# phazei/ComfyUI-HunyuanVideo-Foley

Hardware: AMD Instinct MI355X
Metric: audio-sec/sec (5s clip, 50-step Euler, CFG 4.5) (higher is better)
Workload: dtype bf16; 1 GPU; c2: T2A 5 s, 50 Euler steps, CFG 4.5, hunyuanvideo-foley-xxl, bs=1/GPU, bf16 GEMM operands / fp32 accumulate, weight storage none, DAC-VAE fp32 decode to 48 kHz, host-to-host (H2D noise + D2H waveform timed); clips_per_gpu=1, parallelism=dp1, hip_graph=True, progress_callback=False, collectives=0, bundle_bytes=10565004032, rccl_nranks=1

## Files before the change

### comfyui-hunyuanvideo-foley_amd/csrc/attention.hip

```cpp
#include <type_traits>

#include "kernels.h"

namespace {


template <int HD> __device__ constexpr float attn_scale() {
  return HD == 128 ? 0.08838834764831845f : HD == 64 ? 0.125f : 0.10206207261596575f;
}

__device__ __forceinline__ void attn_block_coords(const AttnArgs& a, int qtile, int& qt, int& h, int& b) {
  const int nq = (a.Sq + qtile - 1) / qtile;
  const int nwg = nq * a.H * a.Bq;
  int bid = (int)blockIdx.x;
  const int xcd = bid & 7, slot = bid >> 3;
  const int q = nwg >> 3, r = nwg & 7;
  bid = ((xcd < r) ? xcd * (q + 1) : r * (q + 1) + (xcd - r) * q) + slot;
  qt = bid % nq;
  const int bh = bid / nq;
  h = bh % a.H;
  b = bh / a.H;
}

template <typename OutT> struct Pack4Out;
template <> struct Pack4Out<float> {
  static __device__ __forceinline__ void store(float* p, const f32x4 v) { *(f32x4*)p = v; }
};
template <> struct Pack4Out<bf16_t> {
  static __device__ __forceinline__ void store(bf16_t* p, const f32x4 v) {
    uint2 w;
    w.x = pack_bf16x2(v[0], v[1]);
    w.y = pack_bf16x2(v[2], v[3]);
    *(uint2*)p = w;
  }
};

template <> struct Pack4Out<f16_t> {
  static __device__ __forceinline__ void store(f16_t* p, const f32x4 v) {
    uint2 w;
    w.x = pack_f16x2(v[0], v[1]);
    w.y = pack_f16x2(v[2], v[3]);
    *(uint2*)p = w;
  }
};

template <typename OutT, int HD>
__global__ __launch_bounds__(64) void attn_kernel(const AttnArgs a) {
  const int lane = threadIdx.x;
  const int j = lane & 31, kh = lane >> 5;
  const int q0 = blockIdx.x * 32;
  const int h = blockIdx.y, b = blockIdx.z;
  const int bk = b / a.kv_bdiv;
  const float* __restrict__ Q = (const float*)a.q + ((long)(b * a.H + h) * a.Sq) * HD;
  const float* __restrict__ K = (const float*)a.k + ((long)(bk * a.H + h) * a.Skv) * HD;
  const float* __restrict__ V = (const float*)a.v + ((long)(bk * a.H + h) * a.Skv) * HD;
  const float scale = attn_scale<HD>();

  constexpr int HH = HD / 2, NC = HD / 8;
  float qr[HH];
  {
    const int qrow = min(q0 + j, a.Sq - 1);
    const f32x4* p = (const f32x4*)(Q + (long)qrow * HD + kh * HH);
#pragma unroll
    for (int c = 0; c < NC; ++c) {
      const f32x4 v = p[c];
      qr[c * 4 + 0] = v[0]; qr[c * 4 + 1] = v[1]; qr[c * 4 + 2] = v[2]; qr[c * 4 + 3] = v[3];
    }
  }

  constexpr int ND = HD / 32;
  f32x16 o[ND];
#pragma unroll
  for (int d = 0; d < ND; ++d)
#pragma unroll
    for (int e = 0; e < 16; ++e) o[d][e] = 0.f;
  float m_run = -INFINITY, l_run = 0.f;

  for (int kt = 0; kt < a.Skv; kt += 32) {
    f32x16 s;
#pragma unroll
    for (int e = 0; e < 16; ++e) s[e] = 0.f;
    {
      const int krow = min(kt + j, a.Skv - 1);
      const f32x4* p = (const f32x4*)(K + (long)krow * HD + kh * HH);
#pragma unroll
      for (int c = 0; c < NC; ++c) {
        const f32x4 v = p[c];
        s = __builtin_amdgcn_mfma_f32_32x32x2f32(v[0], qr[c * 4 + 0], s, 0, 0, 0);
        s = __builtin_amdgcn_mfma_f32_32x32x2f32(v[1], qr[c * 4 + 1], s, 0, 0, 0);
        s = __builtin_amdgcn_mfma_f32_32x32x2f32(v[2], qr[c * 4 + 2], s, 0, 0, 0);
        s = __builtin_amdgcn_mfma_f32_32x32x2f32(v[3], qr[c * 4 + 3], s, 0, 0, 0);
      }
    }
    float mx = -INFINITY;
#pragma unroll
    for (int e = 0; e < 16; ++e) {
      const int key = kt + (e & 3) + 8 * (e >> 2) + 4 * kh;
      s[e] = (key < a.Skv) ? s[e] * scale : -INFINITY;
      mx = fmaxf(mx, s[e]);
    }
    mx = xhalf_max(mx);
    const float m_new = fmaxf(m_run, mx);
    const float alpha = expf(m_run - m_new);
    float ps = 0.f;
#pragma unroll
    for (int e = 0; e < 16; ++e) {
      s[e] = expf(s[e] - m_new);
      ps += s[e];
    }
    ps = xhalf_sum(ps);
    l_run = l_run * alpha + ps;
    m_run = m_new;
#pragma unroll
    for (int d = 0; d < ND; ++d)
#pragma unroll
      for (int e = 0; e < 16; ++e) o[d][e] *= alpha;
#pragma unroll
    for (int t = 0; t < 16; ++t) {
      const int vrow = min(kt + (t & 3) + 8 * (t >> 2) + 4 * kh, a.Skv - 1);
      const float* vp = V + (long)vrow * HD + j;
#pragma unroll
      for (int d = 0; d < ND; ++d)
        o[d] = __builtin_amdgcn_mfma_f32_32x32x2f32(vp[d * 32], s[t], o[d], 0, 0, 0);
    }
  }

  const int tok = q0 + j;
  if (tok >= a.Sq) return;
  const float inv = 1.0f / l_run;
  OutT* dst;
  if (HD == 64 && a.out_rows) {
    const int orow = a.out_rows[(long)b * a.Sq + tok];
    if ((unsigned)orow >= (unsigned)a.out_nrows) return;
    dst = (OutT*)a.outA + (long)orow * (a.H * HD);
  }
  else if (tok < a.split) dst = (OutT*)a.outA + ((long)b * a.split + tok) * (a.H * HD);
  else dst = (OutT*)a.outB + ((long)b * (a.Sq - a.split) + (tok - a.split)) * (a.H * HD);
  dst += h * HD;
#pragma unroll
  for (int d = 0; d < ND; ++d)
#pragma unroll
    for (int g4 = 0; g4 < 4; ++g4) {
      const int c = d * 32 + 8 * g4 + 4 * kh;
#pragma unroll
      for (int u = 0; u < 4; ++u) dst[c + u] = Cvt<OutT>::to(o[d][g4 * 4 + u] * inv);
    }
}

template <typename T, typename OutT>
__global__ __launch_bounds__(256) void attn_bf16_kernel(const AttnArgs a) {
  constexpr int HD = 128;
  __shared__ float sO[4][3][16][64];
  __shared__ float sM[4][32], sL[4][32];
  const int lane = threadIdx.x & 63, w = threadIdx.x >> 6;
  const int j = lane & 31, kh = lane >> 5;
  int qt, h, b;
  attn_block_coords(a, 32, qt, h, b);
  const int q0 = qt * 32;
  const int bk = b / a.kv_bdiv;
  const T* __restrict__ Q = (const T*)a.q + ((long)(b * a.H + h) * a.Sq) * HD;
  const T* __restrict__ K = (const T*)a.k + ((long)(bk * a.H + h) * a.Skv) * HD;
  const T* __restrict__ VT = (const T*)a.v + ((long)(bk * a.H + h) * HD) * a.vt_pitch;
  const float scale2 = 0.08838834764831845f * 1.4426950408889634f;

  const bool stamp = a.dbg && threadIdx.x == 0;
  if (stamp) a.dbg[(long)blockIdx.x * 8 + 0] = wall_clock64();
  bf16x8 qf[8];
  {
    const T* p = Q + (long)min(q0 + j, a.Sq - 1) * HD + 8 * kh;
#pragma unroll
    for (int s = 0; s < 8; ++s) qf[s] = *(const bf16x8*)(p + 16 * s);
  }
  f32x16 o[4];
#pragma unroll
  for (int d = 0; d < 4; ++d)
#pragma unroll
    for (int e = 0; e < 16; ++e) o[d][e] = 0.f;
  float m_run = -INFINITY, l_run = 0.f;

  const int nt = (a.Skv + 31) >> 5;
  const int t0 = (nt * w) >> 2, t1 = (nt * (w + 1)) >> 2;
  const int pi = 16 * ((j >> 2) & 1) + (j & 3) + 4 * (j >> 3);
  auto tile = [&](int kt, const bf16x8 (&kf)[8], const bf16x8 (&vf)[2][4]) {
    f32x16 s;
#pragma unroll
    for (int e = 0; e < 16; ++e) s[e] = 0.f;
#pragma unroll
    for (int st = 0; st < 8; ++st) s = mfma16<T>(kf[st], qf[st], s);
    float mx = -INFINITY;
#pragma unroll
    for (int e = 0; e < 16; ++e) {
      s[e] = (kt + 16 * kh + e < a.Skv) ? s[e] * scale2 : -INFINITY;
      mx = fmaxf(mx, s[e]);
    }
    mx = xhalf_max(mx);
    const float m_new = fmaxf(m_run, mx);
    float ps = 0.f;
    bf16x8 pb[2];
#pragma unroll
    for (int e = 0; e < 16; ++e) {
      const float pv = __builtin_amdgcn_exp2f(s[e] - m_new);
      ps += pv;
      pb[e >> 3][e & 7] = to_carrier<T>(pv);
    }
    ps = xhalf_sum(ps);
    if (__builtin_amdgcn_ballot_w64(m_new > m_run) != 0) {
      const float alpha = __builtin_amdgcn_exp2f(m_run - m_new);
      l_run *= alpha;
#pragma unroll
      for (int d = 0; d < 4; ++d)
#pragma unroll
        for (int e = 0; e < 16; ++e) o[d][e] *= alpha;
    }
    l_run += ps;
    m_run = m_new;
#pragma unroll
    for (int u = 0; u < 2; ++u)
#pragma unroll
      for (int d = 0; d < 4; ++d) o[d] = mfma16<T>(vf[u][d], pb[u], o[d]);
  };
  auto load_k = [&](int kt, bf16x8 (&kf)[8]) {
    const T* p = K + (long)min(kt + pi, a.Skv - 1) * HD + 8 * kh;
#pragma unroll
    for (int st = 0; st < 8; ++st) kf[st] = *(const bf16x8*)(p + 16 * st);
  };
  auto load_v = [&](int kt, bf16x8 (&vf)[2][4]) {
#pragma unroll
    for (int u = 0; u < 2; ++u)
#pragma unroll
      for (int d = 0; d < 4; ++d) vf[u][d] = *(const bf16x8*)(VT + (long)(d * 32 + j) * a.vt_pitch + kt + 16 * kh + 8 * u);
  };
  if (t1 - t0 <= 2) {
    bf16x8 k0[8], k1[8], v0[2][4], v1[2][4];
// ... 13 lines not shown
  } else {
    for (int t = t0; t < t1; ++t) {
      bf16x8 kf[8], vf[2][4];
      load_k(t * 32, kf);
      load_v(t * 32, vf);
      tile(t * 32, kf, vf);
    }
  }

  if (stamp) a.dbg[(long)blockIdx.x * 8 + 2] = wall_clock64();
  if (kh == 0) {
    sM[w][j] = m_run;
    sL[w][j] = l_run;
  }
#pragma unroll
  for (int d = 0; d < 4; ++d) {
    if (d == w) continue;
    const int slot = d < w ? d : d - 1;
#pragma unroll
    for (int e = 0; e < 16; ++e) sO[w][slot][e][lane] = o[d][e];
  }
  __syncthreads();
  if (stamp) a.dbg[(long)blockIdx.x * 8 + 3] = wall_clock64();
  float mstar = -INFINITY;
#pragma unroll
  for (int x = 0; x < 4; ++x) mstar = fmaxf(mstar, sM[x][j]);
  float wt[4], L = 0.f;
#pragma unroll
  for (int x = 0; x < 4; ++x) {
    wt[x] = __builtin_amdgcn_exp2f(sM[x][j] - mstar);
    L += wt[x] * sL[x][j];
  }
  const int tok = q0 + j;
  if (tok >= a.Sq) return;
  const float inv = 1.0f / L;
  OutT* dst;
  if (tok < a.split) dst = (OutT*)a.outA + ((long)b * a.split + tok) * (a.H * HD);
  else dst = (OutT*)a.outB + ((long)b * (a.Sq - a.split) + (tok - a.split)) * (a.H * HD);
  dst += h * HD + w * 32;
  const int slot_mine = 0;
  (void)slot_mine;
  auto finish = [&](auto wc) {
    constexpr int W = decltype(wc)::value;
    float part[3][16];
#pragma unroll
    for (int x = 0, n = 0; x < 4; ++x) {
      if (x == W) continue;
      const int slot = W < x ? W : W - 1;
#pragma unroll
      for (int e = 0; e < 16; ++e) part[n][e] = sO[x][slot][e][lane];
      ++n;
    }
#pragma unroll
    for (int g4 = 0; g4 < 4; ++g4) {
      f32x4 r;
#pragma unroll
      for (int u = 0; u < 4; ++u) {
        const int e = g4 * 4 + u;
        float acc = 0.f;
#pragma unroll
        for (int x = 0, n = 0; x < 4; ++x) {
          if (x == W) acc += wt[x] * o[W][e];
          else acc += wt[x] * part[n++][e];
        }
        r[u] = acc * inv;
      }
      Pack4Out<OutT>::store(dst + 8 * g4 + 4 * kh, r);
    }
  };
  switch (__builtin_amdgcn_readfirstlane(w)) {
    case 0: finish(std::integral_constant<int, 0>{}); break;
    case 1: finish(std::integral_constant<int, 1>{}); break;
    case 2: finish(std::integral_constant<int, 2>{}); break;
    default: finish(std::integral_constant<int, 3>{}); break;
  }
  if (stamp) a.dbg[(long)blockIdx.x * 8 + 4] = wall_clock64();
}

__device__ __forceinline__ void attn_buf_lds16(const void* base, unsigned bytes, unsigned char* lds_wave_base, int voff) {
  const __amdgpu_buffer_rsrc_t r = __builtin_amdgcn_make_buffer_rsrc((void*)base, 0, (int)bytes, 0x00020000);
  __builtin_amdgcn_raw_ptr_buffer_load_lds(r, (__attribute__((address_space(3))) void*)lds_wave_base, 16, voff, 0, 0, 0);
}

template <typename T, typename OutT>
__global__ __launch_bounds__(256) void attn_lds_kernel(const AttnArgs a, const int merge_off) {
  constexpr int HD = 128;
  extern __shared__ __attribute__((aligned(16))) unsigned char dsm[];
  float (*sO)[3][16][64] = (float (*)[3][16][64])(dsm + merge_off);
  float (*sM)[32] = (float (*)[32])(dsm + merge_off + 4 * 3 * 16 * 64 * 4);
  float (*sL)[32] = (float (*)[32])(dsm + merge_off + 4 * 3 * 16 * 64 * 4 + 4 * 32 * 4);
  const int lane = threadIdx.x & 63, w = threadIdx.x >> 6;
  const int j = lane & 31, kh = lane >> 5;
  int qt, h, b;
  attn_block_coords(a, 32, qt, h, b);
  const int q0 = qt * 32;
  const int bk = b / a.kv_bdiv;
  const T* __restrict__ Q = (const T*)a.q + ((long)(b * a.H + h) * a.Sq) * HD;
  const T* __restrict__ K = (const T*)a.k + ((long)(bk * a.H + h) * a.Skv) * HD;
  const T* __restrict__ VT = (const T*)a.v + ((long)(bk * a.H + h) * HD) * a.vt_pitch;
  const float scale2 = 0.08838834764831845f * 1.4426950408889634f;

  const bool stamp = a.dbg && threadIdx.x == 0;
  if (stamp) a.dbg[(long)blockIdx.x * 8 + 0] = wall_clock64();
  const int nt = (a.Skv + 31) >> 5;
  const int lgCV = a.vt_pitch > 128 ? 5 : 4;
  unsigned char* const Ks = dsm;
  unsigned char* const Vs = Ks + nt * 32 * 256;
  unsigned char* const Qs = Vs + (128 << (lgCV + 4));
  const int wv = __builtin_amdgcn_readfirstlane(w);
  {
    const int r4 = lane >> 4, c16 = lane & 15;
    for (int p = wv; p < nt * 8; p += 4) {
      const int row = 4 * p + r4;
      const int g = c16 ^ ((row & 7) | ((row >> 1) & 8));
      attn_buf_lds16(K, (unsigned)a.Skv * 256u, Ks + p * 1024, row * 256 + g * 16);
    }
    const int vchunks = a.vt_pitch >> 3;
    for (int p = wv; p < (128 << lgCV) >> 6; p += 4) {
      const int pos = p * 64 + lane;
      const int row = pos >> lgCV, g = (pos & ((1 << lgCV) - 1)) ^ (row & 15);
      attn_buf_lds16(VT, (unsigned)(HD * a.vt_pitch * 2), Vs + p * 1024, g < vchunks ? (row * a.vt_pitch + g * 8) * 2 : 0x7ffffff0);
    }
    for (int p = wv; p < 8; p += 4) {
      const int row = 4 * p + r4;
      attn_buf_lds16(Q + (long)q0 * HD, (unsigned)(a.Sq - q0) * 256u, Qs + p * 1024, row * 256 + ((c16 ^ (row & 15)) << 4));
    }
  }
  asm volatile("s_waitcnt vmcnt(0)" ::: "memory");
  __syncthreads();
  if (stamp) a.dbg[(long)blockIdx.x * 8 + 1] = wall_clock64();
  bf16x8 qf[8];
#pragma unroll
  for (int s = 0; s < 8; ++s) qf[s] = *(const bf16x8*)(Qs + j * 256 + (((2 * s + kh) ^ (j & 15)) << 4));
  f32x16 o[4];
#pragma unroll
  for (int d = 0; d < 4; ++d)
#pragma unroll
    for (int e = 0; e < 16; ++e) o[d][e] = 0.f;
  float m_run = -INFINITY, l_run = 0.f;

  const int t0 = (nt * w) >> 2, t1 = (nt * (w + 1)) >> 2;
  const int pi = 16 * ((j >> 2) & 1) + (j & 3) + 4 * (j >> 3);
  auto tile = [&](int kt, const bf16x8 (&kf)[8], const bf16x8 (&vf)[2][4]) {
    f32x16 s;
#pragma unroll
    for (int e = 0; e < 16; ++e) s[e] = 0.f;
#pragma unroll
    for (int st = 0; st < 8; ++st) s = mfma16<T>(kf[st], qf[st], s);
    float mx = -INFINITY;
#pragma unroll
    for (int e = 0; e < 16; ++e) {
      s[e] = (kt + 16 * kh + e < a.Skv) ? s[e] * scale2 : -INFINITY;
      mx = fmaxf(mx, s[e]);
    }
    mx = xhalf_max(mx);
    const float m_new = fmaxf(m_run, mx);
    float ps = 0.f;
    bf16x8 pb[2];
#pragma unroll
    for (int e = 0; e < 16; ++e) {
      const float pv = __builtin_amdgcn_exp2f(s[e] - m_new);
      ps += pv;
      pb[e >> 3][e & 7] = to_carrier<T>(pv);
    }
    ps = xhalf_sum(ps);
    if (__builtin_amdgcn_ballot_w64(m_new > m_run) != 0) {
      const float alpha = __builtin_amdgcn_exp2f(m_run - m_new);
      l_run *= alpha;
// ... 523 lines not shown
      pb[e >> 3][e & 7] = to_carrier<T>(pv);
    }
    ps = xhalf_sum(ps);
    if (__builtin_amdgcn_ballot_w64(m_new > m_run) != 0) {
      const float alpha = __builtin_amdgcn_exp2f(m_run - m_new);
      l_run *= alpha;
#pragma unroll
      for (int d = 0; d < ND; ++d)
#pragma unroll
        for (int e = 0; e < 16; ++e) o[d][e] *= alpha;
    }
    l_run += ps;
    m_run = m_new;
#pragma unroll
    for (int u = 0; u < 2; ++u)
#pragma unroll
      for (int d = 0; d < ND; ++d)
        o[d] = mfma16<T>(*(const bf16x8*)(Vs + (d * 32 + j) * VP + (16 * kh + 8 * u) * 2), pb[u], o[d]);
  };
  gload(0);
  lstore(0);
  __syncthreads();
  for (int t = 0; t < nt; ++t) {
    if (t + 1 < nt) gload(t + 1);
    if (t * KT + 32 * kh2 < a.Skv) {
      qk(t & 1);
      softmax_pv(t, t & 1);
    }
    if (t + 1 < nt) {
      lstore((t + 1) & 1);
      __syncthreads();
    }
  }
  __syncthreads();
  float* xm = (float*)lds + qb * (66 * 64);
  if (kh2 == 1) {
    xm[lane] = m_run;
    xm[64 + lane] = l_run;
#pragma unroll
    for (int d = 0; d < ND; ++d)
#pragma unroll
      for (int v = 0; v < 4; ++v) {
        const f32x4 t4 = {o[d][4 * v], o[d][4 * v + 1], o[d][4 * v + 2], o[d][4 * v + 3]};
        *(f32x4*)(xm + 128 + ((d * 4 + v) * 64 + lane) * 4) = t4;
      }
  }
  __syncthreads();
  if (kh2 == 1) return;
  {
    const float m_b = xm[lane], l_b = xm[64 + lane];
    const float m = fmaxf(m_run, m_b);
    const float fa = __builtin_amdgcn_exp2f(m_run - m), fb = __builtin_amdgcn_exp2f(m_b - m);
    l_run = l_run * fa + l_b * fb;
#pragma unroll
    for (int d = 0; d < ND; ++d)
#pragma unroll
      for (int v = 0; v < 4; ++v) {
        const f32x4 t4 = *(const f32x4*)(xm + 128 + ((d * 4 + v) * 64 + lane) * 4);
#pragma unroll
        for (int e = 0; e < 4; ++e) o[d][4 * v + e] = o[d][4 * v + e] * fa + t4[e] * fb;
      }
  }
  const int tok = q0 + j;
  if (tok >= a.Sq) return;
  const float inv = 1.0f / l_run;
  OutT* dst;
  if (tok < a.split) dst = (OutT*)a.outA + ((long)b * a.split + tok) * (a.H * HD);
  else dst = (OutT*)a.outB + ((long)b * (a.Sq - a.split) + (tok - a.split)) * (a.H * HD);
  dst += h * HD;
#pragma unroll
  for (int d = 0; d < ND; ++d)
#pragma unroll
    for (int g4 = 0; g4 < 4; ++g4) {
      const f32x4 v = {o[d][g4 * 4 + 0] * inv, o[d][g4 * 4 + 1] * inv, o[d][g4 * 4 + 2] * inv, o[d][g4 * 4 + 3] * inv};
      Pack4Out<OutT>::store(dst + d * 32 + 8 * g4 + 4 * kh, v);
    }
}

}

static long long* g_attn_dbg = nullptr;
extern "C" void foley_debug_attn_timeline(void* p) { g_attn_dbg = (long long*)p; }

int launch_attention(const AttnArgs& a_in, int out_dtype, hipStream_t st) {
  AttnArgs a = a_in;
  a.dbg = g_attn_dbg;
  if (a.Sq <= 0 || a.Skv <= 0) return foley_set_err("attention: empty sequence", __FILE__, __LINE__);
  const int hd = a.head_dim > 0 ? a.head_dim : 128;
  if (hd != 128 && hd != 64 && hd != 96) return foley_set_err("attention: head_dim must be 128, 96 or 64", __FILE__, __LINE__);
  if (a.grp_q > 0 || a.grp_kv > 0) {
    if (hd != 64 || !foley_is_half(a.in_dtype) || a.grp_q < 1 || a.grp_kv < 1 || a.kv_bdiv != 1 ||
        (long)((a.Sq + a.grp_q - 1) / a.grp_q) * a.grp_kv > a.Skv)
      return foley_set_err("attention: grouped (block-diagonal) form: head_dim 64, 16-bit operands, every query group's keys inside Skv", __FILE__, __LINE__);
  }
  if (a.out_rows && hd != 64) return foley_set_err("attention: the output row table serves head_dim 64 (the conditioning encoders' kernels)", __FILE__, __LINE__);
  dim3 grid((a.Sq + 31) / 32, a.H, a.Bq), block(64);
  const dim3 grid1(grid.x * grid.y * grid.z);
  if (foley_is_half(a.in_dtype)) {
    if (a.vt_pitch < ((a.Skv + 31) & ~31) || (a.vt_pitch & 7))
      return foley_set_err("attention: V^T pitch must cover Skv rounded up to 32 (multiple of 8)", __FILE__, __LINE__);
    if (out_dtype != a.in_dtype && out_dtype != FOLEY_F32)
      return foley_set_err("attention: 16-bit operands produce the same type or fp32", __FILE__, __LINE__);
    const dim3 gw(((a.Sq + 127) / 128) * a.H * a.Bq);
    const bool wide = (long)gw.x >= 256 || hd != 128, h16 = a.in_dtype == FOLEY_F16, o32 = out_dtype == FOLEY_F32;
    const bool longk = wide && hd == 128 && a.Skv >= 512 && (long)gw.x * 4 <= 2048;
    int pair_nq = 0;
    if (longk) {
      long best = 0;
      for (int nq = 6; nq >= 4; --nq) {
        const long wgs = (long)((a.Sq + 32 * nq - 1) / (32 * nq)) * a.H * a.Bq;
        if (wgs <= 256 && wgs > best) { best = wgs; pair_nq = nq; }
      }
      if (best < 160) pair_nq = 0;
    }
    const int nt = (a.Skv + 31) >> 5;
    const long img = (long)nt * 32 * 256 + (128L << ((a.vt_pitch > 128 ? 5 : 4) + 4)) + 32 * 256, mrg = 4 * 3 * 16 * 64 * 4 + 2 * 4 * 32 * 4;
    const bool staged = !wide && hd == 128 && nt >= 4 && a.vt_pitch <= 256 && img <= 160 * 1024;
    const int merge_off = staged && img + mrg <= 160 * 1024 ? (int)img : 0;
    const size_t lds16 = staged ? (size_t)(merge_off ? img + mrg : (img > mrg ? img : mrg)) : 0;
#define FOLEY_ATTN16(T, O)                                                                         \
    do {                                                                                             \
      if (staged) {                                                                                  \
        static std::atomic<unsigned long long> raised{0};                                            \
        hipError_t e_ = foley_raise_lds((const void*)attn_lds_kernel<T, O>, 160 * 1024, raised);     \
        if (e_ != hipSuccess) return foley_set_err(hipGetErrorString(e_), __FILE__, __LINE__);       \
        FOLEY_LAUNCH((attn_lds_kernel<T, O>), grid1, dim3(256), lds16, st, a, merge_off);            \
      } else                                                                                         \
      if (pair_nq) {                                                                                 \
        static std::atomic<unsigned long long> r4{0}, r5{0}, r6{0};                                  \
        const dim3 gp(((a.Sq + 32 * pair_nq - 1) / (32 * pair_nq)) * a.H * a.Bq);                    \
        hipError_t e_ = hipSuccess;                                                                  \
        if (pair_nq == 6) { e_ = foley_raise_lds((const void*)attn_bf16_pair_kernel<T, O, 6>, 6 * 16896, r6); if (e_ == hipSuccess) FOLEY_LAUNCH((attn_bf16_pair_kernel<T, O, 6>), gp, dim3(768), 6 * 16896, st, a); } \
        else if (pair_nq == 5) { e_ = foley_raise_lds((const void*)attn_bf16_pair_kernel<T, O, 5>, 5 * 16896, r5); if (e_ == hipSuccess) FOLEY_LAUNCH((attn_bf16_pair_kernel<T, O, 5>), gp, dim3(640), 5 * 16896, st, a); } \
        else { e_ = foley_raise_lds((const void*)attn_bf16_pair_kernel<T, O, 4>, 2 * 35840, r4); if (e_ == hipSuccess) FOLEY_LAUNCH((attn_bf16_pair_kernel<T, O, 4>), gp, dim3(512), 2 * 35840, st, a); } \
        if (e_ != hipSuccess) return foley_set_err(hipGetErrorString(e_), __FILE__, __LINE__);       \
      } else                                                                                         \
      if (longk) {                                                                                   \
        static std::atomic<unsigned long long> raised{0};                                            \
        hipError_t e_ = foley_raise_lds((const void*)attn_bf16_long_kernel<T, O>, 2 * 35840, raised); \
        if (e_ != hipSuccess) return foley_set_err(hipGetErrorString(e_), __FILE__, __LINE__);       \
        FOLEY_LAUNCH((attn_bf16_long_kernel<T, O>), gw, dim3(256), 2 * 35840, st, a);                \
      } else                                                                                         \
      if (wide && hd == 64 && a.grp_q > 0) FOLEY_LAUNCH((attn_bf16_wide_kernel<T, O, 64, true>), gw, dim3(256), 0, st, a);  \
      else if (wide && hd == 64) FOLEY_LAUNCH((attn_bf16_wide_kernel<T, O, 64>), gw, dim3(256), 0, st, a);  \
      else if (wide && hd == 96) FOLEY_LAUNCH((attn_bf16_wide_kernel<T, O, 96>), gw, dim3(256), 0, st, a);  \
      else if (wide) FOLEY_LAUNCH((attn_bf16_wide_kernel<T, O, 128>), gw, dim3(256), 0, st, a);        \
      else FOLEY_LAUNCH((attn_bf16_kernel<T, O>), grid1, dim3(256), 0, st, a);                         \
    } while (0)
    if (h16) { if (o32) FOLEY_ATTN16(f16_t, float); else FOLEY_ATTN16(f16_t, f16_t); }
    else { if (o32) FOLEY_ATTN16(bf16_t, float); else FOLEY_ATTN16(bf16_t, bf16_t); }
#undef FOLEY_ATTN16
    hipError_t e2 = hipGetLastError();
    if (e2 != hipSuccess) return foley_set_err(hipGetErrorString(e2), __FILE__, __LINE__);
    return 0;
  }
#define FOLEY_ATTN32(O)                                                          \
  do {                                                                           \
    if (hd == 64) FOLEY_LAUNCH((attn_kernel<O, 64>), grid, block, 0, st, a);     \
    else if (hd == 96) FOLEY_LAUNCH((attn_kernel<O, 96>), grid, block, 0, st, a); \
    else FOLEY_LAUNCH((attn_kernel<O, 128>), grid, block, 0, st, a);             \
  } while (0)
  if (out_dtype == FOLEY_F32) FOLEY_ATTN32(float);
  else if (out_dtype == FOLEY_BF16) FOLEY_ATTN32(bf16_t);
  else if (out_dtype == FOLEY_F16) FOLEY_ATTN32(f16_t);
  else return foley_set_err("attention: bad output dtype", __FILE__, __LINE__);
#undef FOLEY_ATTN32
  hipError_t e = hipGetLastError();
  if (e != hipSuccess) return foley_set_err(hipGetErrorString(e), __FILE__, __LINE__);
  return 0;
}
```

### comfyui-hunyuanvideo-foley_amd/csrc/foley_rt.hip

```cpp
#include "../../include/foley_hip.h"
#include "kernels.h"
#include "gemm_plan.h"

#include <algorithm>
#include <climits>
#include <cmath>
#include <cstdio>
#include <cstdlib>
#include <cstring>
#include <cxxabi.h>
#include <atomic>
#include <mutex>
#include <string>
#include <type_traits>
#include <unordered_map>
#include <vector>

thread_local FoleyProfHook g_foley_prof = {nullptr, nullptr};

static std::mutex g_setup_mutex;

static thread_local std::string g_err;
int foley_set_err(const char* msg, const char* file, int line) {
  const char* base = strrchr(file, '/');
// ... 787 lines not shown
    const int P = ly.P;
    const size_t tab_bytes = (size_t)NI * ly.smod_step * 4;
    bool hoist = f.depth_single > 0 && vh * P <= 64 && tab_bytes <= SMOD_TABLE_CAP;
    const size_t svec_bytes = (size_t)NI * vh * Ls * D * es;
    if (hoist) {
      size_t free_b = 0, total_b = 0;
      if (hipMemGetInfo(&free_b, &total_b) != hipSuccess) { hipGetLastError(); free_b = 0; }
      const size_t held = c->smod_tab.bytes + c->svec_tab.bytes;
      if (tab_bytes + svec_bytes > held && (tab_bytes + svec_bytes - held) > free_b / 2) hoist = false;
    }
    if (hoist && (grow(c->smod_tab, tab_bytes) != 0 || grow(c->svec_tab, svec_bytes) != 0)) {
      hipGetLastError();
      hoist = false;
    }
    if (!hoist && (c->smod_tab.p || c->svec_tab.p)) {
      HIPTRY(hipStreamSynchronize(st));
      release(c->smod_tab);
      release(c->svec_tab);
    }
    if (hoist) {
      for (int it = 0; it < NI; ++it)
        TRY(launch_rows_add_act(c->buf.sync_tok, rb_vec(c->buf.vec_table + (size_t)it * D, 0, nullptr), vh * Ls, D, 1,
                                (char*)c->svec_tab.p + (size_t)it * vh * Ls * D * es, T, st));
      GemmArgs gm = gemm_plain(c->svec_tab.p, NI * vh * P, c->fw.smod, c->smod_tab.p, ly.smod_ld);
      gm.segV = P; gm.segS = Ls;
      TRY(launch_gemm(gm, T, EPI_STORE_F32, 0, st));
    }
    ly.hoisted = hoist;
    ly.mod_per = (ly.allper || !hoist) ? ly.per : 0;
    ly.mod_lead = ly.allper ? -1 : ly.lead;
  }
  {
    std::vector<int> tab((size_t)La);
    HIPTRY(hipMemcpy(tab.data(), pl->sync_gather, (size_t)La * 4, hipMemcpyDeviceToHost));
    const float scale = (float)Ls / (float)La;
    for (int l = 0; l < La; ++l)
      if (tab[l] != rb_nearest_exact(l, scale, Ls)) return FAIL(FOLEY_ERR_INVALID, "plan.sync_gather is not the nearest-exact up-sampling table");
  }
  c->prepared = true;
  return 0;
}

static RowBcast rb_vec(const float* base, long step_stride, const int* step_ptr) {
  return RowBcast{base, 0, 0, 1, 1, step_ptr, step_stride};
}
static RowBcast rb_tok(const float* base, long ld, int rows_per_cfg, int L) {
  return RowBcast{base, ld, 1, rows_per_cfg, L, nullptr, 0, 0, 0.f, 0};
}
static RowBcast rb_up(const float* base, long ld, int rows_per_cfg, int L, int Ls, int per = 0, int lead = -1) {
  RowBcast r{base, ld, 2, rows_per_cfg, L, nullptr, 0, Ls, (float)Ls / (float)L, per, 0, 0};
  if (per > 0) {
    r.dense_from = lead < 0 ? INT_MAX : lead;
    r.dense_base = lead < 0 ? 0 : lead * per;
  }
  return r;
}

static int prof_begin(foley_ctx* c, hipStream_t st, const char* label, double flop, double bytes) {
  if (!c->prof.on) return 0;
  ProfRec r{label, flop, bytes, c->prof.get(), c->prof.get(), nullptr};
  c->prof.recs.push_back(r);
  g_foley_prof = FoleyProfHook{r.e0, r.e1, nullptr};
  return 0;
}
static int prof_end(foley_ctx* c, hipStream_t st) {
  if (!c->prof.on) return 0;
  if (g_foley_prof.e0) {
    g_foley_prof.e0 = nullptr;
    HIPTRY(hipEventRecord(c->prof.recs.back().e0, st));
    HIPTRY(hipEventRecord(c->prof.recs.back().e1, st));
  } else {
    c->prof.recs.back().fn = g_foley_prof.fn;
  }
  return 0;
}
#define PROF(label, flop, bytes, call)            \
  do {                                            \
    TRY(prof_begin(c, st, (label), (flop), (bytes))); \
    TRY(call);                                    \
    TRY(prof_end(c, st));                         \
  } while (0)

enum FwdPart { FWD_ALL = 0, FWD_HEAD, FWD_BODY, FWD_FINAL };

static int run_forward(foley_ctx* c, hipStream_t st, FwdPart part = FWD_ALL) {
  const foley_config& f = c->cfg;
  const foley_plan& pl = c->plan;
  const ForwardW& W = c->fw;
  if (!W.ok) return FAIL(FOLEY_ERR_STATE, "forward weights are not resolved (foley_prepare)");
  auto krot = [&pl](GemmArgs g) {
    g.krot_ok = pl.clips == 1 ? 1 : 0;
    return g;
  };
  const int D = f.hidden, H = f.heads, C = f.latent_dim, T = f.compute_dtype;
  const int ncfg = pl.ncfg, clips = pl.clips, La = pl.La, Lv = pl.Lv, Ls = pl.Ls, Lt = pl.Lt, NI = pl.n_iter;
  const int Bc = ncfg * clips, M = Bc * La, Mv = Bc * Lv, S = La + Lv;
  const RunLayout& ly = c->layout;
  const IterArgs ia = iter_args(c);
  const int th = ly.th, vh = ly.vh, lead = ly.lead;
  const bool bf = foley_is_half(T);
  const size_t es = esize(T);
  const int* sp = c->buf.step_ctr;
  void* const qkv_dst[3] = {c->buf.Q, c->buf.K, c->buf.V};
  auto gf = [](double m, double n, double k) { return 2.0 * m * n * k; };
  auto gb = [&](double m, double n, double k, double out_es) { return (m * k + n * k) * (double)es + m * n * out_es; };
  auto af = [&](double b, double sq, double skv) { return 4.0 * b * H * sq * skv * 128.0; };
  auto ab = [&](double b, double sq, double skv) { return (2.0 * b * H * sq * 128.0 + 2.0 * b * H * skv * 128.0) * (double)es; };

  const FwdPart smod_part = f.depth_triple == 0 ? FWD_HEAD : FWD_BODY;
  if (!ly.hoisted && (part == FWD_ALL || part == smod_part)) {
    if (ly.v_rows && lead > 1)
      TRY(launch_rows_add_act(c->buf.sync_lead_rows, rb_vec(c->buf.vec_table, D, sp), lead * ly.per, D, 1, c->buf.svec, T, st));
    else
      for (int h = 0; h < lead; ++h)
        TRY(launch_rows_add_act(c->buf.sync_tok + (size_t)h * Ls * D, rb_vec(c->buf.vec_table, D, sp), ly.per, D, 1,
                                (char*)c->buf.svec + (size_t)h * ly.per * D * es, T, st));
    if (lead < vh)
      TRY(launch_rows_add_act(c->buf.sync_tok + (size_t)lead * Ls * D, rb_vec(c->buf.vec_table, D, sp), (vh - lead) * Ls, D, 1,
                              (char*)c->buf.svec + (size_t)lead * ly.per * D * es, T, st));
    if (f.depth_single > 0) {
      const double n = (double)ly.smod_ld;
      GemmArgs gm = krot(gemm_plain(c->buf.svec, ly.R, W.smod, c->buf.smod, ly.smod_ld));
      PROF("single.modulation (all blocks, one GEMM)", gf(ly.R, n, D), gb(ly.R, n, D, 4), launch_gemm(gm, T, EPI_STORE_F32, 0, st));
    }
  }

  if (part == FWD_ALL || part == FWD_HEAD) {
    GemmArgs g = krot(gemm_plain(c->buf.xin, M, W.audio_in, c->buf.audio, D));
    g.rb = rb_up(c->buf.sync_tok, D, ly.vdiv * La, La, Ls);
    PROF("audio_embedder", gf(M, D, C), gb(M, D, C, 4), launch_gemm(g, T, EPI_STORE_F32, 0, st));
  }
  auto sm_of = [&](int blk, int chunk) {
    const float* smod_b = (ly.hoisted ? (const float*)c->smod_tab.p : c->buf.smod) + (size_t)blk * 6 * D;
    RowBcast r = rb_up(smod_b + (size_t)chunk * D, ly.smod_ld, ly.vdiv * La, La, Ls, ly.mod_per, ly.mod_lead);
    if (ly.hoisted) {
      r.step_ptr = sp;
      r.step_stride = ly.smod_step;
    }
    return r;
  };
  if (part == FWD_HEAD) {
    const bool tri = f.depth_triple > 0;
    auto tb0 = [&](int chunk) { return rb_vec(c->buf.modtab + (size_t)chunk * D, 9L * D, sp); };
    TRY(launch_cache_probe(c->buf.audio, Bc, La, D, tri ? 1e-6f : 1e-5f, tri ? tb0(0) : sm_of(0, 0), tri ? tb0(1) : sm_of(0, 1),
                           ia.sc_mprev, ia.sc_part, ia.sc_rel, st));
    return 0;
  }
  auto final_layer = [&](const LnPending& pending) -> int {
    PROF("final.layernorm", 0.0, (double)M * D * (4 + 4 + es),
         launch_ln_mod_pending(c->buf.audio, M, D, 1e-6f, rb_none(), rb_none(), c->buf.xn_a, T, pending, st));
    PROF("final.linear", gf(M, C, D), gb(M, C, D, 4), launch_gemm(krot(gemm_plain(c->buf.xn_a, M, W.fin, c->buf.pred, C)), T, EPI_STORE_F32, 0, st));
    return 0;
  };
  if (part == FWD_FINAL) return final_layer(LnPending{});
  if (ly.v_rows)
    TRY(launch_gather_rows(c->buf.v_cond0, c->buf.rep_idx, Bc * Lv, 1, c->vis_src * Lv, D, c->buf.vcond, st));
  else
    TRY(launch_gather_rows(c->buf.v_cond0, c->buf.rep_idx, clips * Lv, ncfg, Lv, D, c->buf.vcond, st));

  LnPending pend[2] = {LnPending{}, LnPending{}};
  const int slab_half = bf ? T : 0;
  auto with_partials = [&](GemmArgs& g, float* slabs) {
    g.partial_half = slab_half ? 1 : 0;
    g.partials = slabs;
    g.partial_stride = (long)g.M * g.N;
    g.partial_cap = PART_CAP;
// ... 17 lines not shown
    auto gated2 = [&](const char* label, const Lin& la, const Lin& lv, bool from_hid, int c_gate) -> int {
      GemmArgs g0 = krot(gemm_plain(from_hid ? ss[0].hid : ss[0].att, ss[0].rows, la, ss[0].x, D));
      GemmArgs g1 = krot(gemm_plain(from_hid ? ss[1].hid : ss[1].att, ss[1].rows, lv, ss[1].x, D));
      g0.rb = tb(0, c_gate);
      g1.rb = tb(1, c_gate);
      with_partials(g0, c->buf.part_a);
      with_partials(g1, c->buf.part_v);
      int ks = 1;
      PROF(label, gf(M + Mv, la.N, la.K), gb(M + Mv, la.N, la.K, 4) + (double)la.N * la.K * es,
           launch_gemm_pair(g0, g1, T, EPI_GATE_RES, st, &ks));
      if (ks > 1) {
        pend[0] = LnPending{c->buf.part_a, ks, g0.partial_stride, la.b, g0.rb, slab_half};
        pend[1] = LnPending{c->buf.part_v, ks, g1.partial_stride, lv.b, g1.rb, slab_half};
      }
      return 0;
    };
    auto split_args = [&](int s, int nK, const float* gq, const float* gk, int rot) {
      return qkv_split_args(c, ss[s].qkv, ss[s].rows, ss[s].L, nK, gq, gk, rot, true, qkv_dst, S, ss[s].tok_off,
                            (bf && nK == 3) ? ly.Sp : 0, 1e-6f);
    };
    {
      TRY(ln2(0, 1));
      GemmArgs g0 = krot(gemm_plain(ss[0].xn, ss[0].rows, w.qkv[0], ss[0].qkv, 3 * D));
      GemmArgs g1 = krot(gemm_plain(ss[1].xn, ss[1].rows, w.qkv[1], ss[1].qkv, 3 * D));
      g0.qs = split_args(0, 3, w.qn[0], w.kn[0], 0);
      g1.qs = split_args(1, 3, w.qn[1], w.kn[1], 1);
      PROF("triple.qkv GEMM + RMSNorm/RoPE head split", gf(M + Mv, 3 * D, D), gb(M + Mv, 3 * D, D, es) + 3.0 * D * D * es,
           launch_gemm_pair(g0, g1, T, EPI_QKV_SPLIT, st));
      AttnArgs a{c->buf.Q, c->buf.K, c->buf.V, Bc, H, S, S, 1, c->buf.att_v, c->buf.att_a, Lv, T, bf ? ly.Sp : 0};
      PROF("triple.self attention", af(Bc, S, S), ab(Bc, S, S), launch_attention(a, T, st));
      TRY(gated2("triple.self proj GEMM (gated residual)", w.proj[0], w.proj[1], false, 2));
    }
    {
      TRY(ln2(3, 4));
      GemmArgs g0 = krot(gemm_plain(ss[0].xn, ss[0].rows, w.cq[0], ss[0].qkv, D));
      GemmArgs g1 = krot(gemm_plain(ss[1].xn, ss[1].rows, w.cq[1], ss[1].qkv, D));
      g0.qs = split_args(0, 1, w.cqn[0], nullptr, 2);
      g1.qs = split_args(1, 1, w.cqn[1], nullptr, 2);
      const int Ltp = ly.Ltp, tdiv = ly.tdiv;
      const size_t offk = (size_t)blk * th * H * Lt * 128 * es;
      const size_t offv = (size_t)blk * th * H * (bf ? Ltp : Lt) * 128 * es;
      int fused = 0;
      if (bf && Lt <= 96 && Ltp >= 96 && !ia.tl_sets) {
        for (int s = 0; s < 2; ++s) {
          QkvSplitArgs& q = s ? g1.qs : g0.qs;
          q.attn_k = (char*)c->buf.txt_k + offk; q.attn_vt = (char*)c->buf.txt_v + offv; q.attn_out = ss[s].att;
          q.attn_skv = Lt; q.attn_pitch = Ltp; q.attn_bdiv = tdiv; q.attn_fused = &fused;
        }
      }
      PROF("triple.cross q GEMM + head split (+ cross attention on small grids)", gf(M + Mv, D, D),
           gb(M + Mv, D, D, es) + 1.0 * D * D * es, launch_gemm_pair(g0, g1, T, EPI_QKV_SPLIT, st));
      if (ia.tl_sets) {
        AttnTimelineArgs ta{c->buf.Q, (char*)c->buf.txt_k + offk, (char*)c->buf.txt_v + offv, ia.tl_a, ia.tl_b,
                            ia.tl_alpha, Bc, H, S, Lt, ia.tl_sets, c->buf.att_v, c->buf.att_a, Lv, T, bf ? Ltp : 0};
        PROF("triple.cross attention (prompt timeline)", 2.0 * af(Bc, S, Lt), 2.0 * ab(Bc, S, Lt), launch_attention_timeline(ta, T, st));
      } else if (!fused) {
        AttnArgs a{c->buf.Q, (char*)c->buf.txt_k + offk, (char*)c->buf.txt_v + offv, Bc, H, S, Lt, tdiv, c->buf.att_v, c->buf.att_a, Lv,
                   T, bf ? Ltp : 0};
        PROF("triple.cross attention", af(Bc, S, Lt), ab(Bc, S, Lt), launch_attention(a, T, st));
      }
      TRY(gated2("triple.cross proj GEMM (gated residual)", w.cproj[0], w.cproj[1], false, 5));
    }
    {
      TRY(ln2(6, 7));
      PROF("triple.mlp fc1 GEMM + GELU", gf(M + Mv, f.mlp_hidden, D), gb(M + Mv, f.mlp_hidden, D, es) + (double)f.mlp_hidden * D * es,
           launch_gemm_pair(krot(gemm_plain(ss[0].xn, ss[0].rows, w.fc1[0], ss[0].hid, f.mlp_hidden)),
                            krot(gemm_plain(ss[1].xn, ss[1].rows, w.fc1[1], ss[1].hid, f.mlp_hidden)), T, EPI_GELU_T, st));
      TRY(gated2("triple.mlp fc2 GEMM (gated residual)", w.fc2[0], w.fc2[1], true, 8));
    }
  }

  const int Hc = f.conv_hidden;
  for (int blk = 0; blk < f.depth_single; ++blk) {
    const SingleW& w = W.s[blk];
    auto sm = [&](int chunk) { return sm_of(blk, chunk); };
    PROF("single.layernorm+modulate (+pending split-K sum)", 0.0, ln_bytes_s,
         launch_ln_mod_pending(c->buf.audio, M, D, 1e-5f, sm(0), sm(1), c->buf.xn_a, T, pend[0], st));
    pend[0] = LnPending{};
    GemmArgs gq = krot(gemm_plain(c->buf.xn_a, M, w.qkv, c->buf.qkv_a, 3 * D));
    gq.qs = qkv_split_args(c, c->buf.qkv_a, M, La, 3, w.qn, w.kn, 2, true, qkv_dst, La, 0, bf ? ly.Lap : 0,
                           1.1920928955078125e-07f);
    PROF("single.qkv GEMM + RMSNorm/RoPE head split", gf(M, 3 * D, D), gb(M, 3 * D, D, es), launch_gemm(gq, T, EPI_QKV_SPLIT, 0, st));
    {
      AttnArgs a{c->buf.Q, c->buf.K, c->buf.V, Bc, H, La, La, 1, c->buf.att_a, c->buf.att_a, 0, T, bf ? ly.Lap : 0};
      PROF("single.self attention", af(Bc, La, La), ab(Bc, La, La), launch_attention(a, T, st));
    }
    {
      GemmArgs g = krot(gemm_conv(c->buf.att_a, M, La, D, 3, 1, w.lin1, c->buf.audio, D));
      g.rb = sm(2);
      with_partials(g, c->buf.part_a);
      int ks = 1;
      PROF("single.linear1 conv3 GEMM (gated residual)", gf(M, D, 3 * D), gb(M, D, 3 * D, 4), launch_gemm(g, T, EPI_GATE_RES, 0, st, &ks));
      if (ks > 1) pend[0] = LnPending{c->buf.part_a, ks, g.partial_stride, w.lin1.b, g.rb, slab_half};
    }
    PROF("single.layernorm+modulate (+pending split-K sum)", 0.0, ln_bytes_s,
         launch_ln_mod_pending(c->buf.audio, M, D, 1e-5f, sm(3), sm(4), c->buf.xn_a, T, pend[0], st));
    pend[0] = LnPending{};
    PROF("single.w1/w3 conv3 GEMM + SiLU gate", gf(M, 2 * Hc, 3 * D), gb(M, 2 * Hc, 3 * D, es) - (double)M * Hc * es,
         launch_gemm(krot(gemm_conv(c->buf.xn_a, M, La, D, 3, 1, w.w13, c->buf.hid_a, Hc)), T, EPI_SILUGATE_T, 0, st));
    {
      GemmArgs g = krot(gemm_conv(c->buf.hid_a, M, La, Hc, 3, 1, w.w2, c->buf.audio, D));
      g.rb = sm(5);
      with_partials(g, c->buf.part_a);
      int ks = 1;
      PROF("single.w2 conv3 GEMM (gated residual)", gf(M, D, 3 * Hc), gb(M, D, 3 * Hc, 4), launch_gemm(g, T, EPI_GATE_RES, 0, st, &ks));
      if (ks > 1) pend[0] = LnPending{c->buf.part_a, ks, g.partial_stride, w.w2.b, g.rb, slab_half};
    }
  }

  return final_layer(pend[0]);
}

static int forward_at(foley_ctx* c, const float* latents, int iter, hipStream_t st) {
  if (!c->prepared) return FAIL(FOLEY_ERR_STATE, "foley_prepare has not been called");
  if (iter < 0 || iter >= c->plan.n_iter) return FAIL(FOLEY_ERR_INVALID, "iteration out of range");
  HIPTRY(hipSetDevice(c->device));
  const foley_plan& pl = c->plan;
  HIPTRY(hipMemcpyAsync(c->buf.step_ctr, &iter, sizeof(int), hipMemcpyHostToDevice, st));
  HIPTRY(hipStreamSynchronize(st));
  TRY(launch_latent_rows(latents, pl.clips, c->cfg.latent_dim, pl.La, pl.ncfg, c->buf.xin, c->cfg.compute_dtype, st));
  return run_forward(c, st);
}

extern "C" int foley_dit_forward(foley_ctx* c, const float* latents, int iter, float* out_rows, void* stream_v) {
  if (!c || !latents || !out_rows) return FAIL(FOLEY_ERR_INVALID, "null argument");
  hipStream_t st = (hipStream_t)stream_v;
  TRY(forward_at(c, latents, iter, st));
  const foley_plan& pl = c->plan;
  HIPTRY(hipMemcpyAsync(out_rows, c->buf.pred, (size_t)pl.ncfg * pl.clips * pl.La * c->cfg.latent_dim * 4, hipMemcpyDeviceToDevice, st));
  return 0;
}

extern "C" int foley_profile_forward(foley_ctx* c, const float* latents, int iter, int repeats, foley_prof_entry* out,
                                     int cap, int* n_out, float* bracket_ms, void* stream_v) {
  if (!c || !latents || !out || !n_out || cap < 1 || repeats < 1) return FAIL(FOLEY_ERR_INVALID, "bad argument");
  hipStream_t st = (hipStream_t)stream_v;
  TRY(forward_at(c, latents, iter, st));
  c->prof.recs.clear();
  c->prof.used = 0;
  c->prof.on = true;
  int rc = 0;
  for (int r = 0; r < repeats && rc == 0; ++r) rc = run_forward(c, st);
  c->prof.on = false;
  g_foley_prof = FoleyProfHook{nullptr, nullptr, nullptr};
  if (rc) return rc;
  constexpr int NCAL = 32;
  hipEvent_t cal[2 * NCAL];
  for (int i = 0; i < 2 * NCAL; ++i) cal[i] = c->prof.get();
  for (int i = 0; i < NCAL; ++i) {
    HIPTRY(hipEventRecord(cal[2 * i], st));
    HIPTRY(hipEventRecord(cal[2 * i + 1], st));
  }
  HIPTRY(hipStreamSynchronize(st));
  double cal_ms = 0.0;
  for (int i = 0; i < NCAL; ++i) {
    float ms = 0.f;
    HIPTRY(hipEventElapsedTime(&ms, cal[2 * i], cal[2 * i + 1]));
    cal_ms += ms;
  }
  if (bracket_ms) *bracket_ms = (float)(cal_ms / NCAL);
  int n = 0;
  for (const ProfRec& r : c->prof.recs) {
    float ms = 0.f;
    HIPTRY(hipEventElapsedTime(&ms, r.e0, r.e1));
    int j = 0;
    for (; j < n; ++j)
      if (!strcmp(out[j].label, r.label)) break;
    if (j == n) {
      if (n == cap) return FAIL(FOLEY_ERR_INVALID, "profile: entry buffer too small");
      memset(&out[n], 0, sizeof(out[n]));
      strncpy(out[n].label, r.label, sizeof(out[n].label) - 1);
      if (r.fn) {
        const char* mangled = hipKernelNameRefByPtr(r.fn, st);
// ... 531 lines not shown
  g.out_shift = d->out_shift; g.out_check = d->out_check; g.rb = to_rb(&d->rb); g.res = d->res;
  g.alpha = d->alpha; g.alphaC = d->alphaC > 0 ? d->alphaC : 1;
  g.ksplit = d->ksplit;
  g.rstride = d->rstride;
  g.ldw = d->ldw;
  g.wfmt = d->wfmt;
  g.gelu_erf = d->gelu_erf;
  if (d->partials) {
    if (d->partial_slabs < 1) return FAIL(FOLEY_ERR_INVALID, "partials need partial_slabs >= 1");
    g.partials = d->partials; g.partial_stride = (long)d->M * d->N; g.partial_cap = d->partial_slabs;
    g.partial_half = d->partial_dtype != 0;
    if (d->partial_dtype != 0 && d->partial_dtype != d->dtype) return FAIL(FOLEY_ERR_INVALID, "partial_dtype must be 0 (fp32) or the operand dtype");
  }
  if (g.segV < 1 || g.segS < 1 || g.osegV < 1 || g.taps < 1) return FAIL(FOLEY_ERR_INVALID, "bad GEMM descriptor");
  if (d->epilogue == EPI_QKV_SPLIT) {
    const foley_qkv_split_desc* q = d->qkv;
    if (!q) return FAIL(FOLEY_ERR_INVALID, "epilogue 7 needs a head-split descriptor");
    QkvSplitArgs& a = g.qs;
    a.qkv = nullptr; a.M = d->M; a.L = q->L; a.H = q->H; a.nK = q->nK;
    for (int i = 0; i < 3; ++i) { a.gain[i] = q->gain[i]; a.pos[i] = q->pos[i]; a.dst[i] = q->dst[i]; }
    a.S_tot = q->S_tot; a.tok_off = q->tok_off; a.out_dtype = q->out_dtype; a.vt_pitch = q->vt_pitch;
    a.eps = q->eps; a.cos_tab = q->cos_tab; a.sin_tab = q->sin_tab;
    a.attn_k = q->attn_k; a.attn_vt = q->attn_vt; a.attn_out = q->attn_out;
    a.attn_skv = q->attn_skv; a.attn_pitch = q->attn_pitch; a.attn_bdiv = q->attn_bdiv; a.attn_fused = q->attn_fused;
    if (q->attn_fused) *q->attn_fused = 0;
  }
  return 0;
}

static thread_local int g_gemm_krot_ok = 0;
extern "C" int foley_debug_gemm_krot(int on) {
  const int prev = g_gemm_krot_ok;
  g_gemm_krot_ok = on ? 1 : 0;
  return prev;
}

extern "C" int foley_op_gemm(const foley_gemm_desc* d, void* stream) {
  GemmArgs g;
  if (int rc = gemm_args_of(d, g)) return rc;
  g.zeros = zero_page();
  g.krot_ok = g_gemm_krot_ok;
  int ks = 1;
  const int rc = launch_gemm(g, d->dtype, d->epilogue, d->tile, (hipStream_t)stream, &ks);
  if (d->ksplit_used) *d->ksplit_used = ks;
  return rc;
}

static int gemm_pair_args_of(const foley_gemm_desc* d0, const foley_gemm_desc* d1, GemmArgs& g0, GemmArgs& g1) {
  if (!d0 || !d1) return FAIL(FOLEY_ERR_INVALID, "null descriptor");
  if (d0->dtype != d1->dtype || d0->epilogue != d1->epilogue)
    return FAIL(FOLEY_ERR_INVALID, "GEMM pair: the two problems must share the operand dtype and the epilogue");
  if (d0->tile != 0 || d1->tile != 0) return FAIL(FOLEY_ERR_INVALID, "GEMM pair: the pair launcher picks its own tile (tile must be 0)");
  if (int rc = gemm_args_of(d0, g0)) return rc;
  return gemm_args_of(d1, g1);
}

extern "C" int foley_debug_gemm_pair(const foley_gemm_desc* d0, const foley_gemm_desc* d1, void* stream) {
  GemmArgs g0, g1;
  if (int rc = gemm_pair_args_of(d0, d1, g0, g1)) return rc;
  g0.zeros = g1.zeros = zero_page();
  g0.krot_ok = g1.krot_ok = g_gemm_krot_ok;
  int ks = 1;
  const int rc = launch_gemm_pair(g0, g1, d0->dtype, d0->epilogue, (hipStream_t)stream, &ks);
  if (d0->ksplit_used) *d0->ksplit_used = ks;
  return rc;
}

extern "C" int foley_debug_gemm_plan(const foley_gemm_desc* d0, const foley_gemm_desc* d1, int krot_ok, int32_t out[4]) {
  if (!out) return FAIL(FOLEY_ERR_INVALID, "null output");
  GemmArgs g0, g1;
  if (int rc = d1 ? gemm_pair_args_of(d0, d1, g0, g1) : gemm_args_of(d0, g0)) return rc;
  GemmPlan p;
  switch (d0->dtype) {
    case FOLEY_F32: p = plan_gemm<float>(g0, d1 ? &g1 : nullptr, d0->epilogue, d0->tile, krot_ok); break;
    case FOLEY_BF16: p = plan_gemm<bf16_t>(g0, d1 ? &g1 : nullptr, d0->epilogue, d0->tile, krot_ok); break;
    case FOLEY_F16: p = plan_gemm<f16_t>(g0, d1 ? &g1 : nullptr, d0->epilogue, d0->tile, krot_ok); break;
    default: return FAIL(FOLEY_ERR_INVALID, "GEMM: unsupported operand dtype");
  }
  if (p.err) return FAIL(FOLEY_ERR_INVALID, p.err);
  out[0] = p.tile; out[1] = p.ksplit; out[2] = p.n_groups; out[3] = p.k_rot;
  return 0;
}

extern "C" int foley_op_attention_hd(const void* q, const void* k, const void* v, int in_dtype, int vt_pitch, int Bq,
                                     int H, int Sq, int Skv, int kv_bdiv, void* outA, void* outB, int split,
                                     int out_dtype, int head_dim, void* stream) {
  AttnArgs a{q, k, v, Bq, H, Sq, Skv, kv_bdiv > 0 ? kv_bdiv : 1, outA, outB, split, in_dtype, vt_pitch, head_dim};
  return launch_attention(a, out_dtype, (hipStream_t)stream);
}

extern "C" int foley_op_attention_scatter(const void* q, const void* k, const void* v, int in_dtype, int vt_pitch, int G, int H, int Sq,
                                          int Skv, int grp_q, int grp_kv, const int32_t* out_rows, void* out, int out_nrows, int out_dtype, void* stream) {
  if (!out_rows || !out) return FAIL(FOLEY_ERR_INVALID, "null argument");
  if (out_nrows < 1) return FAIL(FOLEY_ERR_INVALID, "attention_scatter: out has no rows");
  AttnArgs a{q, k, v, G, H, Sq, Skv, 1, out, out, 0, in_dtype, vt_pitch, 64};
  a.grp_q = grp_q; a.grp_kv = grp_kv;
  a.out_rows = out_rows;
  a.out_nrows = out_nrows;
  return launch_attention(a, out_dtype, (hipStream_t)stream);
}

extern "C" int foley_op_attention(const void* q, const void* k, const void* v, int in_dtype, int vt_pitch, int Bq,
                                  int H, int Sq, int Skv, int kv_bdiv, void* outA, void* outB, int split,
                                  int out_dtype, void* stream) {
  return foley_op_attention_hd(q, k, v, in_dtype, vt_pitch, Bq, H, Sq, Skv, kv_bdiv, outA, outB, split, out_dtype, 128, stream);
}

extern "C" int foley_op_attention_timeline(const void* q, const void* k, const void* v, int in_dtype, int vt_pitch, int Bq, int H, int Sq,
                                           int Skv, int n_sets, const int32_t* set_a, const int32_t* set_b, const float* alpha, void* outA,
                                           void* outB, int split, int out_dtype, void* stream) {
  AttnTimelineArgs a{q, k, v, set_a, set_b, alpha, Bq, H, Sq, Skv, n_sets, outA, outB, split, in_dtype, vt_pitch};
  return launch_attention_timeline(a, out_dtype, (hipStream_t)stream);
}

extern "C" int foley_op_qkv_regroup(const void* qkv, int n_rows, int dtype, int H, const int32_t* idx_q, int G, int Sq, const int32_t* idx_kv, int Skv,
                                    void* q, void* k, void* v, int vt_pitch, void* stream) {
  if (!qkv || !idx_q || !idx_kv || !q || !k || !v) return FAIL(FOLEY_ERR_INVALID, "null argument");
  return launch_qkv_regroup(qkv, n_rows, dtype, H, idx_q, G, Sq, idx_kv, Skv, q, k, v, vt_pitch, (hipStream_t)stream);
}

extern "C" int foley_op_resample_sinc(const float* x, int B, int N, int orig, int new_rate, const float* taps, int ntaps, int width,
                                      float* out, int Nout, void* stream) {
  if (!x || !taps || !out) return FAIL(FOLEY_ERR_INVALID, "null argument");
  return launch_resample_sinc(x, B, N, orig, new_rate, taps, ntaps, width, out, Nout, (hipStream_t)stream);
}

extern "C" int foley_op_logmel(const float* w16, int B, int N16, const float* basis, const int32_t* mel_lo, const int32_t* mel_len,
                               const float* mel_w, int mel_wp, void* patches, int out_dtype, float* mel_out, void* stream) {
  if (!w16 || !basis || !mel_lo || !mel_len || !mel_w || !patches) return FAIL(FOLEY_ERR_INVALID, "null argument");
  return launch_logmel(w16, B, N16, basis, mel_lo, mel_len, mel_w, mel_wp, patches, out_dtype, mel_out, (hipStream_t)stream);
}

extern "C" int foley_op_loudness_energy(const float* x, int B, int C, int N, int64_t ld, const double* T16, double* work,
                                        int64_t work_doubles, double* e, void* stream) {
  if (!x || !T16) return FAIL(FOLEY_ERR_INVALID, "null argument");
  return launch_loudness_energy(x, B, C, N, (long)ld, T16, work, work_doubles, e, (hipStream_t)stream);
}

extern "C" int foley_op_loudness_gate(const double* e, int B, int C, int nh, double* lufs, double* gamma, double* block_lufs,
                                      void* stream) {
  return launch_loudness_gate(e, B, C, nh, lufs, gamma, block_lufs, (hipStream_t)stream);
}

extern "C" int foley_op_true_peak(const float* x, int B, int C, int N, int64_t ld, const float* taps36, float* true_peak,
                                  float* sample_peak, float* envelope, void* stream) {
  if (!x || !taps36 || !true_peak) return FAIL(FOLEY_ERR_INVALID, "null argument");
  return launch_true_peak(x, B, C, N, (long)ld, taps36, true_peak, sample_peak, envelope, (hipStream_t)stream);
}

extern "C" int foley_op_loudness_apply(const float* x, int B, int C, int N, int64_t ld, const float* gain, int limiter,
                                       double ceiling, int lookahead, const float* taps36, float* y, int64_t ldy, float* g_out,
                                       void* stream) {
  if (!x || !gain || !y) return FAIL(FOLEY_ERR_INVALID, "null argument");
  return launch_loudness_apply(x, B, C, N, (long)ld, gain, limiter, ceiling, lookahead, taps36, y, (long)ldy, g_out,
                               (hipStream_t)stream);
}

extern "C" int foley_op_resize_aa_u8(const uint8_t* in, long outer, int len_in, long inner, int len_out, const int32_t* xmin,
                                     const int32_t* xsize, const int16_t* weights, int kmax, int precision, uint8_t* out, void* stream) {
  if (!in || !xmin || !xsize || !weights || !out) return FAIL(FOLEY_ERR_INVALID, "null argument");
  return launch_resize_aa_u8(in, outer, len_in, inner, len_out, xmin, xsize, weights, kmax, precision, out, (hipStream_t)stream);
}

extern "C" int foley_op_ln_mod(const float* x, int M, int D, float eps, const foley_rowbcast* shift,
                               const foley_rowbcast* scale, void* out, int out_dtype, void* stream) {
  return launch_ln_mod(x, M, D, eps, to_rb(shift), to_rb(scale), out, out_dtype, (hipStream_t)stream);
// ... 255 lines not shown
```

### comfyui-hunyuanvideo-foley_amd/csrc/gemm_conv3.hip

```cpp
#include "gemm_common.h"

namespace {

template <typename T, int BM, int BN, int WM, int WN, int NS, int EPI>
__global__ __launch_bounds__(WM* WN * 64) void gemm_conv3_kernel(const GemmPair pr) {
  const int sel = (int)blockIdx.x >= pr.tiles0 ? 1 : 0;
  const GemmArgs& g = pr.g[sel];
  constexpr int NT = WM * WN * 64;
  constexpr int EPC = Frag<T>::EPC;
  constexpr int BK = 8 * EPC;
  constexpr int TM = BM / WM, TN = BN / WN, FM = TM / 32, FN = TN / 32;
  constexpr int AROWS = BM + 2, WROWS = 3 * BN;
  constexpr int RA = (AROWS * 8 + NT - 1) / NT;
  constexpr int RB = (WROWS * 8) / NT;
  static_assert((WROWS * 8) % NT == 0, "bad tile");
  constexpr int STAGE = (AROWS + WROWS) * LDS_PITCH;
  static_assert(EPI != EPI_SILUGATE_T || (FN % 2 == 0), "gated epilogue needs fragment pairs");
  extern __shared__ __attribute__((aligned(16))) unsigned char lds[];

  const int tiles_m = (g.M + BM - 1) / BM;
  const int tiles_n = (g.N + BN - 1) / BN;
  int bid = (int)blockIdx.x - (sel ? pr.tiles0 : 0);
  {
    const int nwg = tiles_m * tiles_n * (EPI == EPI_GATE_RES ? g.ksplit : 1);
    const int xcd = bid & 7, slot = bid >> 3;
    const int q = nwg >> 3, r = nwg & 7;
    bid = ((xcd < r) ? xcd * (q + 1) : r * (q + 1) + (xcd - r) * q) + slot;
  }
  int ks = 0;
  if constexpr (EPI == EPI_GATE_RES) {
    ks = bid % g.ksplit;
    bid /= g.ksplit;
  }
  const int tm = bid % tiles_m, tn = bid / tiles_m;
  const int m0 = tm * BM, n0 = tn * BN;
  const int tid = threadIdx.x, lane = tid & 63, wave = tid >> 6;
  tl_stamp(g, 0);
  const int wm = wave / WN, wn = wave % WN;
  const int C = g.tapC;

  const T* ap[RA];
  int a_lds[RA];
  bool a_use[RA];
#pragma unroll
  for (int i = 0; i < RA; ++i) {
    const int c = tid + i * NT;
    a_use[i] = c < AROWS * 8;
    const int rl = a_use[i] ? (c >> 3) : 0;
    int r = m0 - 1 + rl;
    r = r < 0 ? 0 : (r >= g.M ? g.M - 1 : r);
    ap[i] = (const T*)g.A + (long)r * g.lda + (c & 7) * EPC;
    a_lds[i] = rl * LDS_PITCH + (c & 7) * 16;
  }
  const T* wp[RB];
  int w_lds[RB];
  bool w_ok[RB];
#pragma unroll
  for (int i = 0; i < RB; ++i) {
    const int c = tid + i * NT;
    const int rl = c >> 3;
    const int tap = rl / BN, nl = rl - tap * BN;
    const int n = n0 + nl;
    w_ok[i] = n < g.N;
    wp[i] = (const T*)g.W + (long)(w_ok[i] ? n : 0) * g.K + (long)tap * C + (c & 7) * EPC;
    w_lds[i] = (AROWS + rl) * LDS_PITCH + (c & 7) * 16;
  }

  u32x4 ra[NS][RA], rw[NS][RB];
  const u32x4 zero4 = {0u, 0u, 0u, 0u};
  f32x16 acc[FM][FN];
#pragma unroll
  for (int i = 0; i < FM; ++i)
#pragma unroll
    for (int j = 0; j < FN; ++j)
#pragma unroll
      for (int e = 0; e < 16; ++e) acc[i][j][e] = 0.f;

  const int fi = lane & 31, kh = lane >> 5;
  bool zl[FM], zr[FM];
#pragma unroll
  for (int i = 0; i < FM; ++i) {
    const int r = m0 + wm * TM + i * 32 + fi;
    const int q = r % g.segV;
    zl[i] = q == 0;
    zr[i] = q == g.segV - 1;
  }

  int kc_begin = 0, nkc = C / BK;
  if constexpr (EPI == EPI_GATE_RES) {
    const int tot = nkc;
    kc_begin = (int)((long)tot * ks / g.ksplit);
    nkc = (int)((long)tot * (ks + 1) / g.ksplit) - kc_begin;
  }
  int ld_c0 = kc_begin * BK;

#define FOLEY_GLOAD3(slot)                                                                  \
  {                                                                                         \
    _Pragma("unroll") for (int i = 0; i < RA; ++i) ra[slot][i] = *(const u32x4*)(ap[i] + ld_c0); \
    _Pragma("unroll") for (int i = 0; i < RB; ++i) rw[slot][i] = *(const u32x4*)(wp[i] + ld_c0); \
    ld_c0 += BK;                                                                            \
  }

#pragma unroll
  for (int s = 0; s < NS - 1; ++s)
    if (s < nkc) FOLEY_GLOAD3(s);

  for (int kt0 = 0; kt0 < nkc; kt0 += NS) {
#pragma unroll
    for (int j = 0; j < NS; ++j) {
      const int kt = kt0 + j;
      if (kt < nkc) {
        if (kt + NS - 1 < nkc) FOLEY_GLOAD3((j + NS - 1) % NS);
        unsigned char* St = lds + (kt & 1) * STAGE;
#pragma unroll
        for (int i = 0; i < RA; ++i)
          if (a_use[i]) *(u32x4*)(St + a_lds[i]) = ra[j][i];
#pragma unroll
// ... 122 lines not shown
```

### comfyui-hunyuanvideo-foley_amd/csrc/gemm_impl.h

```cpp
#pragma once
#include "gemm_plan.h"

extern long long* g_gemm_dbg;
extern int g_gemm_dbg_mode;
extern thread_local int g_gemm_last[3];

namespace {

template <typename T, int BM, int BN, int WM, int WN, int NS, int EPI, bool CONV>
__global__ __launch_bounds__(WM* WN * 64) void gemm_kernel(const GemmPair pr) {
  const int sel = (int)blockIdx.x >= pr.tiles0 ? 1 : 0;
  const GemmArgs& g = pr.g[sel];
  constexpr int NT = WM * WN * 64;
  constexpr int EPC = Frag<T>::EPC;
  constexpr int BK = 8 * EPC;
  constexpr int RPP = NT / 8;
  constexpr int TM = BM / WM, TN = BN / WN, FM = TM / 32, FN = TN / 32;
  constexpr int RA = BM / RPP, RB = BN / RPP;
  constexpr int STAGE = (BM + BN) * LDS_PITCH;
  static_assert(BM % RPP == 0 && BN % RPP == 0 && TM % 32 == 0 && TN % 32 == 0, "bad tile");
  static_assert(EPI != EPI_SILUGATE_T || (FN % 2 == 0), "gated epilogue needs fragment pairs");

  extern __shared__ __attribute__((aligned(16))) unsigned char lds[];

  const int tiles_m = (g.M + BM - 1) / BM;
  const int tiles_n = (g.N + BN - 1) / BN;
  int bid = (int)blockIdx.x - (sel ? pr.tiles0 : 0);
  {
    const int nwg = tiles_m * tiles_n * (EPI == EPI_GATE_RES ? g.ksplit : 1);
    const int xcd = bid & 7, slot = bid >> 3;
    const int q = nwg >> 3, r = nwg & 7;
    bid = ((xcd < r) ? xcd * (q + 1) : r * (q + 1) + (xcd - r) * q) + slot;
  }
  int ks = 0;
  if constexpr (EPI == EPI_GATE_RES) {
    ks = bid % g.ksplit;
    bid /= g.ksplit;
  }
  const int tm = bid % tiles_m, tn = bid / tiles_m;
  const int m0 = tm * BM, n0 = tn * BN;
  const int tid = threadIdx.x, lane = tid & 63, wave = tid >> 6;
  tl_stamp(g, 0);
  const int wm = wave / WN, wn = wave % WN;
  const int chunk = tid & 7, lrow = tid >> 3;

  const T* ap[RA];
  int a_q[RA];
  bool a_ok[RA];
#pragma unroll
  for (int i = 0; i < RA; ++i) {
    const int r = m0 + lrow + i * RPP;
    a_ok[i] = r < g.M;
    const int rr = a_ok[i] ? r : 0;
    int b = 0, q = rr;
    if constexpr (CONV) {
      b = rr / g.segV;
      q = rr - b * g.segV;
    }
    const int qs = q * (g.rstride > 1 ? g.rstride : 1);
    ap[i] = (const T*)g.A + ((long)b * g.segS + qs) * g.lda + chunk * EPC;
    a_q[i] = qs;
  }
  const T* wp[RB];
  bool w_ok[RB];
#pragma unroll
  for (int i = 0; i < RB; ++i) {
    const int n = n0 + lrow + i * RPP;
    w_ok[i] = n < g.N;
    wp[i] = (const T*)g.W + (long)(w_ok[i] ? n : 0) * g.K + chunk * EPC;
  }

  u32x4 ra[NS][RA], rw[NS][RB];
  const u32x4 zero4 = {0u, 0u, 0u, 0u};
  constexpr bool DUAL = (FM * FN == 1) && sizeof(T) == 2;
  f32x16 acc2;
  if constexpr (DUAL) {
#pragma unroll
    for (int e = 0; e < 16; ++e) acc2[e] = 0.f;
  }
  f32x16 acc[FM][FN];
#pragma unroll
  for (int i = 0; i < FM; ++i)
#pragma unroll
    for (int j = 0; j < FN; ++j)
#pragma unroll
      for (int e = 0; e < 16; ++e) acc[i][j][e] = 0.f;

  const int fi = lane & 31, kh = lane >> 5;
  int kt_begin = 0, nk = g.K / BK;
  if constexpr (EPI == EPI_GATE_RES) {
    const int tot = nk;
    kt_begin = (int)((long)tot * ks / g.ksplit);
    nk = (int)((long)tot * (ks + 1) / g.ksplit) - kt_begin;
  }
  const long tap_step = (long)g.dil * g.lda;
  int ld_k0 = kt_begin * BK;
  int ld_c0 = ld_k0, ld_toff = g.tap0;
  if (kt_begin > 0) {
    const int tap = ld_k0 / g.tapC;
    ld_c0 = ld_k0 - tap * g.tapC;
    ld_toff = g.tap0 + tap * g.dil;
  }
  long ld_roff = (long)ld_toff * g.lda;
  int wr_c0 = ld_c0, wr_toff = ld_toff;

#define FOLEY_GLOAD(slot)                                                                  \
  {                                                                                        \
    _Pragma("unroll") for (int i = 0; i < RA; ++i) {                                       \
      if constexpr (CONV) {                                                                \
        const bool in_ = (unsigned)(a_q[i] + ld_toff) < (unsigned)g.segS;                  \
        ra[slot][i] = *(const u32x4*)(ap[i] + (in_ ? ld_roff : 0L) + ld_c0);               \
      } else {                                                                             \
        ra[slot][i] = *(const u32x4*)(ap[i] + ld_k0);                                      \
      }                                                                                    \
    }                                                                                      \
    _Pragma("unroll") for (int i = 0; i < RB; ++i) rw[slot][i] = *(const u32x4*)(wp[i] + ld_k0); \
    ld_k0 += BK;                                                                           \
    if constexpr (CONV) {                                                                  \
      ld_c0 += BK;                                                                         \
      if (ld_c0 >= g.tapC) {                                                               \
        ld_c0 = 0;                                                                         \
        ld_toff += g.dil;                                                                  \
// ... 47 lines not shown
#pragma unroll
          for (int jj = 0; jj < FN; ++jj) {
            const unsigned char* p = Bs + (wn * TN + jj * 32 + fi) * LDS_PITCH + kh * 64;
#pragma unroll
            for (int c = 0; c < 4; ++c) {
              const f32x4 v = *(const f32x4*)(p + c * 16);
              b[jj][c * 4 + 0] = v[0]; b[jj][c * 4 + 1] = v[1]; b[jj][c * 4 + 2] = v[2]; b[jj][c * 4 + 3] = v[3];
            }
          }
#pragma unroll
          for (int s = 0; s < 16; ++s)
#pragma unroll
            for (int i = 0; i < FM; ++i)
#pragma unroll
              for (int jj = 0; jj < FN; ++jj)
                acc[i][jj] = __builtin_amdgcn_mfma_f32_32x32x2f32(a[i][s], b[jj][s], acc[i][jj], 0, 0, 0);
        } else {
#pragma unroll
          for (int s = 0; s < 4; ++s) {
            bf16x8 a[FM], b[FN];
#pragma unroll
            for (int i = 0; i < FM; ++i)
              a[i] = *(const bf16x8*)(As + (wm * TM + i * 32 + fi) * LDS_PITCH + s * 32 + kh * 16);
#pragma unroll
            for (int jj = 0; jj < FN; ++jj)
              b[jj] = *(const bf16x8*)(Bs + (wn * TN + jj * 32 + fi) * LDS_PITCH + s * 32 + kh * 16);
            if constexpr (DUAL) {
              if (s & 1) acc2 = mfma16<T>(a[0], b[0], acc2);
              else acc[0][0] = mfma16<T>(a[0], b[0], acc[0][0]);
            } else {
#pragma unroll
              for (int i = 0; i < FM; ++i)
#pragma unroll
                for (int jj = 0; jj < FN; ++jj)
                  acc[i][jj] = mfma16<T>(a[i], b[jj], acc[i][jj]);
            }
          }
        }
      }
    }
  }
#undef FOLEY_GLOAD
  if constexpr (DUAL) {
#pragma unroll
    for (int e = 0; e < 16; ++e) acc[0][0][e] += acc2[e];
  }

  tl_stamp(g, 2);
  if constexpr (EPI == EPI_QKV_SPLIT) {
    gemm_epilogue_qkv<T, BM, BN, WM, WN>(g, acc, lds, m0, n0);
  } else {
    if (g.vec_out) gemm_epilogue_lds<T, EPI, BM, BN, WM, WN>(g, acc, lds, m0, n0, ks);
    else gemm_epilogue<T, EPI, FM, FN, TM, TN>(g, acc, m0, n0, wm, wn, fi, kh, ks);
  }
  tl_stamp(g, 3);
}

__device__ __forceinline__ void glds16(const void* gptr, unsigned char* lds_wave_base) {
  __builtin_amdgcn_global_load_lds((const __attribute__((address_space(1))) void*)gptr,
                                   (__attribute__((address_space(3))) void*)lds_wave_base, 16, 0, 0);
}

__device__ __forceinline__ void buf_lds16(const void* base, unsigned bytes, unsigned char* lds_wave_base, int voff, int soff) {
  const __amdgpu_buffer_rsrc_t r = __builtin_amdgcn_make_buffer_rsrc((void*)base, 0, (int)bytes, 0x00020000);
  __builtin_amdgcn_raw_ptr_buffer_load_lds(r, (__attribute__((address_space(3))) void*)lds_wave_base, 16, voff, soff, 0, 0);
}

template <typename T, int BM, int BN, int WM, int WN, int NS, int EPI>
__global__ __launch_bounds__(WM* WN * 64) void gemm_glds_kernel(const GemmPair pr) {
  const int sel = (int)blockIdx.x >= pr.tiles0 ? 1 : 0;
  const GemmArgs& g = pr.g[sel];
  constexpr int NW = WM * WN;
  constexpr int EPC = Frag<T>::EPC;
  constexpr int BK = 8 * EPC;
  constexpr int TM = BM / WM, TN = BN / WN, FM = TM / 32, FN = TN / 32;
  constexpr int AI = BM / 8 / NW, BI = BN / 8 / NW;
  constexpr int STAGE = (BM + BN) * 128;
  static_assert(BM % (8 * NW) == 0 && BN % (8 * NW) == 0, "bad tile");
  static_assert(EPI != EPI_SILUGATE_T || (FN % 2 == 0), "gated epilogue needs fragment pairs");
  extern __shared__ __attribute__((aligned(16))) unsigned char lds[];

  const int tiles_m = (g.M + BM - 1) / BM;
  const int tiles_n = (g.N + BN - 1) / BN;
  int bid = (int)blockIdx.x - (sel ? pr.tiles0 : 0);
  {
    const int nwg = tiles_m * tiles_n * (EPI == EPI_GATE_RES ? g.ksplit : 1);
    const int xcd = bid & 7, slot = bid >> 3;
    const int q = nwg >> 3, r = nwg & 7;
    bid = ((xcd < r) ? xcd * (q + 1) : r * (q + 1) + (xcd - r) * q) + slot;
  }
  int ks = 0;
  if constexpr (EPI == EPI_GATE_RES) {
    ks = bid % g.ksplit;
    bid /= g.ksplit;
  }
  const int tm = bid % tiles_m, tn = bid / tiles_m;
  const int m0 = tm * BM, n0 = tn * BN;
  const int tid = threadIdx.x, lane = tid & 63, wave = tid >> 6;
  tl_stamp(g, 0);
  const int wm = wave / WN, wn = wave % WN;
  const int lr = lane >> 3, lp = lane & 7;

  constexpr int ESZ = (int)sizeof(T);
  constexpr int OOB = 0x7ffffff0;
  int a_base[AI], a_q[AI], vA[AI];
#pragma unroll
  for (int i = 0; i < AI; ++i) {
    const int rl = (wave * AI + i) * 8 + lr;
    const int r = m0 + rl;
    const int rr = r < g.M ? r : 0;
    const int b = g.segV >= g.M ? 0 : rr / g.segV, q = rr - b * g.segV;
    const int qs = q * (g.rstride > 1 ? g.rstride : 1);
    a_base[i] = r < g.M ? (int)((((long)b * g.segS + qs) * g.lda + (lp ^ ((rl >> 1) & 7)) * EPC) * ESZ) : -1;
    a_q[i] = qs;
  }
  int vW[BI];
#pragma unroll
  for (int i = 0; i < BI; ++i) {
    const int rl = (wave * BI + i) * 8 + lr;
    const int n = n0 + rl;
    vW[i] = (n < g.N) ? (int)(((long)n * g.K + (lp ^ ((rl >> 1) & 7)) * EPC) * ESZ) : OOB;
  }
  auto set_tap = [&](int toff) {
#pragma unroll
    for (int i = 0; i < AI; ++i) {
      const bool in = a_base[i] >= 0 && (unsigned)(a_q[i] + toff) < (unsigned)g.segS;
      vA[i] = in ? a_base[i] + toff * (int)(g.lda * ESZ) : OOB;
    }
  };

  f32x16 acc[FM][FN];
#pragma unroll
  for (int i = 0; i < FM; ++i)
#pragma unroll
    for (int j = 0; j < FN; ++j)
#pragma unroll
      for (int e = 0; e < 16; ++e) acc[i][j][e] = 0.f;

  const int fi = lane & 31, kh = lane >> 5;
  int kt_begin = 0, nk = g.K / BK;
  if constexpr (EPI == EPI_GATE_RES) {
    const int tot = nk;
    kt_begin = (int)((long)tot * ks / g.ksplit);
    nk = (int)((long)tot * (ks + 1) / g.ksplit) - kt_begin;
  }
  int ld_k0 = kt_begin * BK;
  int ld_c0 = ld_k0, ld_toff = g.tap0;
  if (kt_begin > 0) {
    const int tap = ld_k0 / g.tapC;
    ld_c0 = ld_k0 - tap * g.tapC;
    ld_toff = g.tap0 + tap * g.dil;
  }
  set_tap(ld_toff);

  auto issue = [&](int stage) {
    unsigned char* As = lds + stage * STAGE;
    unsigned char* Bs = As + BM * 128;
    const int sA = ld_c0 * ESZ, sW = ld_k0 * ESZ;
#pragma unroll
    for (int i = 0; i < AI; ++i)
      buf_lds16(g.A, g.a_bytes, As + (wave * AI + i) * 1024, vA[i], sA);
#pragma unroll
    for (int i = 0; i < BI; ++i)
      buf_lds16(g.W, g.w_bytes, Bs + (wave * BI + i) * 1024, vW[i], sW);
    ld_k0 += BK;
    ld_c0 += BK;
    if (ld_c0 >= g.tapC) {
      ld_c0 = 0;
      ld_toff += g.dil;
      set_tap(ld_toff);
    }
  };

#pragma unroll
  for (int s = 0; s < NS - 1; ++s)
    if (s < nk) issue(s);

  int a_row[FM], a_sw[FM], b_row[FN], b_sw[FN];
#pragma unroll
// ... 195 lines not shown
```

### comfyui-hunyuanvideo-foley_amd/csrc/gemm_plan.h

```cpp
#pragma once
#include "gemm_common.h"

namespace {

enum TileFamily : unsigned char { FAM_NONE, FAM_REG, FAM_GLDS, FAM_WS8, FAM_WS4, FAM_HEAD, FAM_CONV3, FAM_WSCONV3, FAM_WIDE };

struct TileInfo {
  short bm, bn;
  TileFamily fam;
  bool fp8;
  bool ldw;
  bool head;
  bool chunks;
  bool grouped;
  short ks_target;
  char per_cu;
  char reg_twin;
  char scalar_twin;
};

constexpr TileInfo kTiles[33] = {
     {},
     {128, 128, FAM_REG,     0, 0, 1, 0, 0, 192, 1, 0, 0},
     {64,  128, FAM_REG,     0, 0, 1, 0, 0, 768, 1, 0, 0},
     {64,  64,  FAM_REG,     0, 0, 0, 0, 0, 768, 3, 0, 0},
     {128, 64,  FAM_REG,     0, 0, 0, 0, 0, 768, 1, 0, 0},
     {128, 128, FAM_GLDS,    0, 0, 1, 0, 0, 192, 1, 1, 0},
     {64,  64,  FAM_GLDS,    0, 0, 0, 0, 0, 768, 3, 3, 0},
     {128, 128, FAM_GLDS,    0, 0, 1, 0, 0, 192, 1, 1, 0},
     {64,  128, FAM_GLDS,    0, 0, 1, 0, 0, 768, 1, 2, 0},
     {256, 128, FAM_GLDS,    0, 0, 1, 0, 0, 192, 1, 1, 0}, {},
     {128, 128, FAM_CONV3,   0, 0, 0, 1, 0, 192, 1, 0, 0}, {},
     {64,  64,  FAM_CONV3,   0, 0, 0, 1, 0, 512, 3, 0, 0}, {},
     {128, 128, FAM_WS8,     1, 1, 1, 0, 1, 192, 1, 1, 0}, {}, {}, {},
     {256, 128, FAM_WS8,     1, 1, 1, 0, 1, 192, 1, 1, 0}, {},
     {128, 128, FAM_WSCONV3, 1, 1, 0, 1, 1, 192, 1, 0, 0},
     {256, 64,  FAM_WSCONV3, 0, 1, 0, 1, 0, 192, 1, 0, 0},
     {256, 128, FAM_WSCONV3, 1, 1, 0, 1, 1, 192, 1, 0, 0},
     {192, 128, FAM_WSCONV3, 0, 1, 0, 1, 1, 192, 1, 0, 0},
     {128, 128, FAM_WS4,     0, 1, 1, 0, 1, 192, 1, 1, 15},
     {96,  128, FAM_HEAD,    0, 1, 1, 0, 0, 768, 1, 1, 0},
     {64,  128, FAM_HEAD,    0, 1, 1, 0, 0, 768, 1, 2, 0},
     {192, 128, FAM_HEAD,    0, 1, 1, 0, 1, 768, 1, 1, 0},
     {256, 128, FAM_WS4,     0, 1, 1, 0, 1, 192, 1, 1, 19}, {},
     {256, 256, FAM_WIDE,    1, 1, 0, 1, 1, 192, 1, 0, 0},
     {256, 256, FAM_WIDE,    1, 1, 1, 0, 1, 192, 1, 0, 0},
};

inline const TileInfo& tile_info(int tile) {
  static constexpr TileInfo none{};
  return tile >= 0 && tile < 33 ? kTiles[tile] : none;
}

struct GemmPlan {
  int tile = 0, ksplit = 1, n_groups = 0, k_rot = 0;
  int vec_out[2] = {0, 0};
  bool attn_fused = false;
  const char* err = nullptr;
};

template <typename T>
const char* check_args(const GemmArgs& g) {
  constexpr int BK = 8 * Frag<T>::EPC;
  if (g.K % BK || g.tapC % BK || g.taps * g.tapC != g.K || g.lda % Frag<T>::EPC)
    return "GEMM: K / tap width / lda must be multiples of the 128-byte K-slice";
  if (((uintptr_t)g.A | (uintptr_t)g.W) & 15) return "GEMM: operands must be 16-byte aligned";
  if (g.partial_half && sizeof(T) != 2) return "GEMM: 16-bit partial slabs need 16-bit operands";
  if (g.wfmt && sizeof(T) != 2) return "GEMM: fp8 weight storage needs bf16 operands";
  return nullptr;
}

template <typename T>
const char* check_qkv_split(const GemmArgs& q) {
  const QkvSplitArgs& s = q.qs;
  if (s.nK < 1 || s.nK > 3 || s.H < 1 || q.N != s.nK * s.H * 128 || s.L < 1 || q.M % s.L)
    return "fused head split: N must be nK*H*128 and M a multiple of L";
  if (s.out_dtype != DtCode<T>::v) return "fused head split: output dtype must equal the operand dtype";
  if (s.vt_pitch && (sizeof(T) != 2 || s.vt_pitch % 8 || (s.tok_off + s.L) > s.vt_pitch))
    return "fused head split: bad transposed-V pitch";
  uintptr_t al = (uintptr_t)s.cos_tab | (uintptr_t)s.sin_tab | (uintptr_t)q.bias;
  for (int i = 0; i < s.nK; ++i) {
    if (!s.dst[i]) return "fused head split: null destination";
    al |= (uintptr_t)s.dst[i] | (uintptr_t)s.gain[i] | (uintptr_t)s.rcos[i] | (uintptr_t)s.rsin[i];
    if (s.pos[i] && (!s.cos_tab || !s.sin_tab)) return "fused head split: RoPE tables missing";
    if ((s.rcos[i] != nullptr) != (s.rsin[i] != nullptr) || (s.rcos[i] && !s.pos[i]))
      return "fused head split: gathered rotation rows need both tables and a position table";
// ... 141 lines not shown
      if (g1) n += (long)((g1s.M + bm - 1) / bm) * ((g1s.N + bn - 1) / bn);
      return n;
    };
    if (plain(g) && (!g1 || plain(g1s))) {
      const double cur = (double)((tiles(tile == 28 ? 192 : 256, 128) + 255) / 256) * (tile == 28 ? 0.86 : 1.0);
      const double wide = (double)((tiles(256, 256) + 255) / 256) * 1.64;
      if (wide < 0.95 * cur) tile = 32;
    }
  }
  if (epi != EPI_GATE_RES || g.ksplit == 1 || (g.ksplit == 0 && sizeof(T) == 4)) {
    g.ksplit = 1;
  } else if (g.ksplit == 0) {
    const TileInfo& ti = tile_info(tile);
    if (ti.bm == 0) return fail("GEMM: unknown tile");
    const long blocks = (long)((g.M + ti.bm - 1) / ti.bm) * ((g.N + ti.bn - 1) / ti.bn);
    const int nk = ti.chunks ? g.tapC / BK : g.K / BK;
    long want = (ti.ks_target + blocks - 1) / blocks;
    if (want > nk / 12) want = nk / 12;
    if (deferred) {
      long both = blocks;
      if (g1) both += (long)((g1->M + ti.bm - 1) / ti.bm) * ((g1->N + ti.bn - 1) / ti.bn);
      want = 256L * ti.per_cu / both;
      if (tile == 21 && both > 256) want = both < 512 ? 2 : 1;
      if (want > nk / 4) want = nk / 4;
    }
    g.ksplit = (int)(want < 1 ? 1 : (want > 16 ? 16 : want));
  }
  if (epi == EPI_GATE_RES && g.partials) {
    int cap = g.partial_cap;
    if (g1 && g1s.partial_cap < cap) cap = g1s.partial_cap;
    if (g1 && !g1s.partials) cap = 1;
    if (g.ksplit > cap) g.ksplit = cap < 1 ? 1 : cap;
  }
  g1s.ksplit = g.ksplit;
  if (!fits) {
    if (g.wfmt) return fail("GEMM: fp8-weight operands exceed the 2 GiB buffer-offset range");
    if (tile_info(tile).fam == FAM_WSCONV3) return fail("GEMM: conv3 operands exceed the 2 GiB buffer-offset range");
    if (tile_info(tile).fam == FAM_WIDE) return fail("GEMM: the 256x256 tiles range every load against 32-bit buffer extents: operands exceed the 2 GiB buffer-offset range");
    if (tile_info(tile).reg_twin) tile = tile_info(tile).reg_twin;
  }
  const TileInfo& ti = tile_info(tile);
  {
    if (ti.grouped && g.M >= 1536 && !g1) {
      const long tm_ = (g.M + ti.bm - 1) / ti.bm, tn_ = (g.N + ti.bn - 1) / ti.bn;
      if (tm_ * tn_ * (epi == EPI_GATE_RES ? g.ksplit : 1) > 256 && tn_ >= 2) {
        int pg = 1;
        while ((pg + 1) * (pg + 1) * ti.bn <= 32 * ti.bm) ++pg;
        const int n = (int)((tn_ + pg / 2) / pg);
        plan.n_groups = n < 1 ? 1 : n;
      }
    }
  }
  {
    const int rbm = (ti.fam == FAM_WS8 || ti.fam == FAM_WS4 || ti.fam == FAM_HEAD) ? ti.bm : 0;
    if (krot_ok && rbm && sizeof(T) == 2 && g.taps == 1 && (!g1 || g1s.taps == 1)) {
      const long ks_ = epi == EPI_GATE_RES ? g.ksplit : 1;
      long n = (long)((g.M + rbm - 1) / rbm) * ((g.N + 127) / 128) * ks_;
      if (g1) n += (long)((g1s.M + rbm - 1) / rbm) * ((g1s.N + 127) / 128) * ks_;
      if (n <= 256 && (g.M + rbm - 1) / rbm >= 2) plan.k_rot = 1;
    }
  }
  plan.vec_out[0] = gemm_vec_out_ok<T>(g, epi) ? 1 : 0;
  if (g1) plan.vec_out[1] = gemm_vec_out_ok<T>(g1s, epi) ? 1 : 0;
  if (ti.scalar_twin && epi != EPI_QKV_SPLIT && !(plan.vec_out[0] && (!g1 || plan.vec_out[1]))) tile = ti.scalar_twin;
  if (ti.fam == FAM_HEAD && (epi != EPI_QKV_SPLIT || g.wfmt)) return fail("GEMM: tile 27 (64x128) serves the fused head split with bf16 weights only");
  if ((g.ldw != g.K || (g1 && g1s.ldw != g1s.K)) && !tile_info(tile).ldw)
    return fail("GEMM: padded weight rows (ldw != K) need a wave-specialised tile");
  if (tile_info(tile).fam == FAM_NONE) return fail("GEMM: bad tile id");
  if (epi == EPI_QKV_SPLIT) {
    auto fuses = [](const GemmArgs& q) {
      const QkvSplitArgs& s = q.qs;
      return s.attn_out && s.attn_k && s.attn_vt && s.nK == 1 && s.vt_pitch == 0 && s.attn_skv >= 1 && s.attn_skv <= 96 &&
             s.attn_pitch >= 96 && s.attn_pitch % 8 == 0 && s.attn_bdiv >= 1 &&
             ((long)s.L * s.attn_bdiv >= 64 || q.M <= 2L * s.L * s.attn_bdiv) &&
             !(((uintptr_t)s.attn_k | (uintptr_t)s.attn_vt | (uintptr_t)s.attn_out) & 15);
    };
    plan.attn_fused = sizeof(T) == 2 && tile == 27 && fuses(g) && (!g1 || fuses(g1s));
  }
  plan.tile = tile;
  plan.ksplit = g.ksplit;
  return plan;
}

}
```

### comfyui-hunyuanvideo-foley_amd/csrc/gemm_wide_impl.h

```cpp
#pragma once
#include "gemm_ws_impl.h"

namespace {

constexpr int wide_inflight(int nsb, int taps, int tap, int ai, int bi) {
  int n = 0;
  for (int j = 1; j <= nsb - 2; ++j) n += bi + (((tap + j) % taps == 0) ? ai : 0);
  return n;
}

template <int N> __device__ __forceinline__ void wide_wait_vm() { asm volatile("s_waitcnt vmcnt(%0)" ::"n"(N) : "memory"); }

template <typename T, int NW, int TAPS, int NSB, int NAB, int EPI, int WF, int SEL>
__device__ __forceinline__ void gemm_wide_body(const GemmPair& pr) {
  const GemmArgs& g = pr.g[SEL];
  constexpr int BM = 256, BN = 256, BK = 32, ESZ = 2, OOB = 0x7ffffff0;
  constexpr int WM = 2, WN = NW / 2, TM = BM / WM, TN = BN / WN, FM = TM / 32, FN = TN / 32;
  constexpr int WSZ = WF ? 1 : 2, BROW = BK * WSZ;
  constexpr int APC = 16 + (TAPS == 3 ? 1 : 0);
  constexpr int ABUF = APC * 1024;
  constexpr int APW = 16 / NW;
  constexpr int BSL = BN * BROW;
  constexpr int BPW = BSL / 1024 / NW;
  constexpr int ZROW = 258;
  constexpr int DUMMY = NAB * ABUF + NSB * BSL;
  constexpr int AIW = APW + (TAPS == 3 ? 1 : 0);
  static_assert(NW == 8, "two waves per SIMD (a four-wave form with 128x128 wave tiles - one wave per SIMD, nothing to alternate with - was built and measured: w1/w3 at M = 4000 296 us against 249)");
  static_assert(TAPS == 1 || TAPS == 3, "plain linear or conv k=3");
  static_assert(BPW >= 1 && APW >= 1, "bad tile");
  static_assert(TAPS * NAB >= NSB - 1 + TAPS, "an activation buffer would be refilled while its chunk is still being consumed");
  static_assert(wide_inflight(NSB, TAPS, 0, AIW, BPW) < 64, "vmcnt is a 6-bit counter");
  static_assert(EPI != EPI_SILUGATE_T || (FN % 2 == 0), "gated epilogue needs fragment pairs");
  extern __shared__ __attribute__((aligned(16))) unsigned char lds[];

  const int tiles_m = (g.M + BM - 1) / BM;
  const int tiles_n = (g.N + BN - 1) / BN;
  int bid = (int)blockIdx.x - (SEL ? pr.tiles0 : 0);
  {
    const int nwg = tiles_m * tiles_n * (EPI == EPI_GATE_RES ? g.ksplit : 1);
    const int xcd = bid & 7, slot = bid >> 3;
    const int q = nwg >> 3, r = nwg & 7;
    bid = ((xcd < r) ? xcd * (q + 1) : r * (q + 1) + (xcd - r) * q) + slot;
  }
  int ks = 0;
  if constexpr (EPI == EPI_GATE_RES) {
    const int tiles = tiles_m * tiles_n;
    ks = bid / tiles;
    bid -= ks * tiles;
  }
  int tm, tn;
  tile_coords(bid, tiles_m, tiles_n, g.n_groups, tm, tn);
  const int m0 = tm * BM, n0 = tn * BN;
  const int tid = threadIdx.x, lane = tid & 63;
  const int wave = __builtin_amdgcn_readfirstlane(tid >> 6);
  tl_stamp(g, 0);
  const int C = g.tapC;
  int kc_begin = 0, nkc = C / BK;
  if constexpr (EPI == EPI_GATE_RES) {
    const int tot = nkc;
    kc_begin = (int)((long)tot * ks / g.ksplit);
    nkc = (int)((long)tot * (ks + 1) / g.ksplit) - kc_begin;
  }
  const int nk = TAPS * nkc;

  const int lr = lane >> 2, lp = lane & 3;
  int vA[APW];
#pragma unroll
  for (int i = 0; i < APW; ++i) {
    const int j = (wave * APW + i) * 16 + lr;
    const int r = m0 + j;
    vA[i] = r < g.M ? (int)((unsigned)r * (unsigned)(g.lda * ESZ) + (unsigned)((lp ^ ((j >> 2) & 3)) * 16)) : OOB;
  }
  int vH = OOB;
  const bool halo_wave = TAPS == 3 && wave == NW - 1;
  if constexpr (TAPS == 3) {
    const int r = lr == 0 ? m0 - 1 : (lr == 1 ? m0 + BM : -1);
    if (halo_wave && r >= 0 && r < g.M) vH = (int)((unsigned)r * (unsigned)(g.lda * ESZ) + (unsigned)(lp * 16));
  }
  int vW[BPW];
#pragma unroll
  for (int i = 0; i < BPW; ++i) {
    if constexpr (WF == 0) {
      const int rl = (wave * BPW + i) * 16 + lr;
      const int n = n0 + rl;
      vW[i] = (n < g.N) ? (int)((unsigned)n * (unsigned)(g.ldw * ESZ) + (unsigned)((lp ^ ((rl >> 2) & 3)) * 16)) : OOB;
    } else {
      const int rl = (wave * BPW + i) * 32 + (lane >> 1);
      const int n = n0 + rl;
      vW[i] = (n < g.N) ? (int)((unsigned)n * (unsigned)g.ldw + (unsigned)(((lane & 1) ^ ((rl >> 3) & 1)) * 16)) : OOB;
    }
  }
  int is_ch = kc_begin * BK, is_ab = 0, is_bs = 0, is_n = 0;
  auto issue = [&](int tapc) {
    const bool valid = is_n < nk;
    if (tapc == 0) {
      unsigned char* Ab = lds + is_ab * ABUF;
      const int sA = valid ? is_ch * ESZ : OOB;
#pragma unroll
      for (int i = 0; i < APW; ++i) buf_lds16(g.A, g.a_bytes, Ab + (wave * APW + i) * 1024, vA[i], sA);
      if constexpr (TAPS == 3) buf_lds16(g.A, g.a_bytes, halo_wave ? Ab + 16 * 1024 : lds + DUMMY, vH, sA);
      is_ab = is_ab + 1 == NAB ? 0 : is_ab + 1;
    }
    unsigned char* Bs = lds + NAB * ABUF + is_bs * BSL;
    const int sW = valid ? (tapc * C + is_ch) * WSZ : OOB;
#pragma unroll
    for (int i = 0; i < BPW; ++i) buf_lds16(g.W, g.w_bytes, Bs + (wave * BPW + i) * 1024, vW[i], sW);
    is_bs = is_bs + 1 == NSB ? 0 : is_bs + 1;
    ++is_n;
    if (tapc == TAPS - 1) is_ch += BK;
  };
#pragma unroll
  for (int s = 0; s < NSB - 1; ++s) issue(s % TAPS);

  const int wm = wave / WN, wn = wave % WN;
  const int fi = lane & 31, kh = lane >> 5;
  f32x16 acc[FM][FN];
#pragma unroll
  for (int i = 0; i < FM; ++i)
#pragma unroll
    for (int j = 0; j < FN; ++j)
#pragma unroll
      for (int e = 0; e < 16; ++e) acc[i][j][e] = 0.f;
  int a_ad[2][TAPS][FM];
#pragma unroll
  for (int i = 0; i < FM; ++i) {
    const int tr = wm * TM + i * 32 + fi;
#pragma unroll
    for (int t = 0; t < TAPS; ++t) {
      int row = tr;
      if constexpr (TAPS == 3) {
        const int q = (m0 + tr) % g.segV;
        const bool ok = !((t == 0 && q == 0) || (t == 2 && q == g.segV - 1));
        const int s = tr + t - 1;
        row = !ok ? ZROW : (s < 0 ? 256 : (s >= BM ? 257 : s));
// ... 208 lines not shown
```

### comfyui-hunyuanvideo-foley_amd/csrc/gemm_ws_impl.h

```cpp
#pragma once
#include <hip/hip_runtime.h>

#include <type_traits>

#include "common.h"
#include "gemm_common.h"

namespace {

__device__ __forceinline__ void buf_lds16(const void* base, unsigned bytes, unsigned char* lds_wave_base, int voff, int soff) {
  const __amdgpu_buffer_rsrc_t r = __builtin_amdgcn_make_buffer_rsrc((void*)base, 0, (int)bytes, 0x00020000);
  __builtin_amdgcn_raw_ptr_buffer_load_lds(r, (__attribute__((address_space(3))) void*)lds_wave_base, 16, voff, soff, 0, 0);
}

__device__ __forceinline__ void tile_coords(int id, int tiles_m, int tiles_n, int n_groups, int& tm, int& tn) {
  if (n_groups <= 0 || n_groups > tiles_n) {
    tm = id % tiles_m;
    tn = id / tiles_m;
    return;
  }
  const int P = tiles_n / n_groups, r = tiles_n % n_groups;
  const int big = r * (P + 1) * tiles_m;
  int pg, p0, local;
  if (id < big) {
    pg = P + 1;
    const int gi = id / (pg * tiles_m);
    local = id - gi * pg * tiles_m;
    p0 = gi * pg;
  } else {
    pg = P;
    const int i2 = id - big, gi = i2 / (pg * tiles_m);
    local = i2 - gi * pg * tiles_m;
    p0 = r * (P + 1) + gi * pg;
  }
  tm = local / pg;
  tn = p0 + local - tm * pg;
}

__device__ __forceinline__ void hard_barrier() {
  __builtin_amdgcn_sched_barrier(0);
  __builtin_amdgcn_s_barrier();
  __builtin_amdgcn_sched_barrier(0);
}

template <int WF, typename T>
__device__ __forceinline__ void cvt_fp8x16(const u32x4 w, bf16x8& lo, bf16x8& hi) {
  uint32_t p[8];
#pragma unroll
  for (int i = 0; i < 4; ++i) {
    if constexpr (__is_same(T, f16_t)) {
      if constexpr (WF == 1) {
        p[2 * i] = __builtin_bit_cast(uint32_t, __builtin_amdgcn_cvt_scalef32_pk_f16_fp8((int)w[i], 1.0f, false));
        p[2 * i + 1] = __builtin_bit_cast(uint32_t, __builtin_amdgcn_cvt_scalef32_pk_f16_fp8((int)w[i], 1.0f, true));
      } else {
        p[2 * i] = __builtin_bit_cast(uint32_t, __builtin_amdgcn_cvt_scalef32_pk_f16_bf8((int)w[i], 1.0f, false));
        p[2 * i + 1] = __builtin_bit_cast(uint32_t, __builtin_amdgcn_cvt_scalef32_pk_f16_bf8((int)w[i], 1.0f, true));
      }
    } else {
      if constexpr (WF == 1) {
        p[2 * i] = __builtin_bit_cast(uint32_t, __builtin_amdgcn_cvt_scalef32_pk_bf16_fp8((int)w[i], 1.0f, false));
        p[2 * i + 1] = __builtin_bit_cast(uint32_t, __builtin_amdgcn_cvt_scalef32_pk_bf16_fp8((int)w[i], 1.0f, true));
      } else {
        p[2 * i] = __builtin_bit_cast(uint32_t, __builtin_amdgcn_cvt_scalef32_pk_bf16_bf8((int)w[i], 1.0f, false));
        p[2 * i + 1] = __builtin_bit_cast(uint32_t, __builtin_amdgcn_cvt_scalef32_pk_bf16_bf8((int)w[i], 1.0f, true));
      }
    }
  }
  const u32x4 l = {p[0], p[1], p[2], p[3]}, h = {p[4], p[5], p[6], p[7]};
  lo = __builtin_bit_cast(bf16x8, l);
  hi = __builtin_bit_cast(bf16x8, h);
}

template <typename T, int BM, int BN, int WM, int WN, int NS, int LW, int EPI, int WF, int SEL>
__device__ __forceinline__ void gemm_ws_body(const GemmPair& pr) {
  constexpr int sel = SEL;
  const GemmArgs& g = pr.g[SEL];
  constexpr int NW = WM * WN;
  constexpr int BK = 64, ESZ = 2, OOB = 0x7ffffff0;
  constexpr int TM = BM / WM, TN = BN / WN, FM = TM / 32, FN = TN / 32;
  constexpr int WSZ = WF ? 1 : 2;
  constexpr int BROW = 64 * WSZ;
  constexpr int AI = BM / 8 / LW, BI = BN * BROW / 1024 / LW;
  constexpr int STAGE = BM * 128 + BN * BROW;
  constexpr bool TWOB = BM == 256 && WM * WN == 8;
  static_assert(BM % (8 * LW) == 0 && (BN * BROW) % (1024 * LW) == 0 && BI >= 1, "bad tile");
  static_assert((NS - 1) * (AI + BI) < 64, "vmcnt is a 6-bit counter");
  static_assert(EPI != EPI_SILUGATE_T || (FN % 2 == 0), "gated epilogue needs fragment pairs");
  extern __shared__ __attribute__((aligned(16))) unsigned char lds[];

  const int tiles_m = (g.M + BM - 1) / BM;
  const int tiles_n = (g.N + BN - 1) / BN;
  int bid = (int)blockIdx.x - (sel ? pr.tiles0 : 0);
  {
    const int nwg = tiles_m * tiles_n * (EPI == EPI_GATE_RES ? g.ksplit : 1);
    const int xcd = bid & 7, slot = bid >> 3;
    const int q = nwg >> 3, r = nwg & 7;
    bid = ((xcd < r) ? xcd * (q + 1) : r * (q + 1) + (xcd - r) * q) + slot;
  }
  int ks = 0;
  if constexpr (EPI == EPI_GATE_RES) {
    const int tiles = tiles_m * tiles_n;
    ks = bid / tiles;
    bid -= ks * tiles;
  }
  int tm, tn;
  tile_coords(bid, tiles_m, tiles_n, g.n_groups, tm, tn);
  const int m0 = tm * BM, n0 = tn * BN;
  const int tid = threadIdx.x, lane = tid & 63;
  const int wave = __builtin_amdgcn_readfirstlane(tid >> 6);
  tl_stamp(g, 0);

  int kt_begin = 0, nk = g.K / BK;
  if constexpr (EPI == EPI_GATE_RES) {
    const int tot = nk;
    kt_begin = (int)((long)tot * ks / g.ksplit);
    nk = (int)((long)tot * (ks + 1) / g.ksplit) - kt_begin;
  }

  if (wave >= NW) {
    const int lw = wave - NW;
    const int lr = lane >> 3, lp = lane & 7;
    int a_base[AI], a_q[AI], vA[AI];
#pragma unroll
    for (int i = 0; i < AI; ++i) {
      const int rl = (lw * AI + i) * 8 + lr;
      const int r = m0 + rl;
      const int rr = r < g.M ? r : 0;
      const int b = g.segV >= g.M ? 0 : rr / g.segV, q = rr - b * g.segV;
      const int qs = q * (g.rstride > 1 ? g.rstride : 1);
      a_base[i] = r < g.M ? (int)((unsigned)(b * g.segS + qs) * (unsigned)(g.lda * ESZ) + (unsigned)((lp ^ ((rl >> 1) & 7)) * 16)) : -1;
      a_q[i] = qs;
    }
    int vW[BI];
#pragma unroll
    for (int i = 0; i < BI; ++i) {
      if constexpr (WF == 0) {
        const int rl = (lw * BI + i) * 8 + lr;
        const int n = n0 + rl;
        vW[i] = (n < g.N) ? (int)((unsigned)n * (unsigned)(g.ldw * ESZ) + (unsigned)((lp ^ ((rl >> 1) & 7)) * 16)) : OOB;
      } else {
        const int rl = (lw * BI + i) * 16 + (lane >> 2);
        const int n = n0 + rl;
        vW[i] = (n < g.N) ? (int)((unsigned)n * (unsigned)g.ldw + (unsigned)(((lane & 3) ^ ((rl >> 2) & 3)) * 16)) : OOB;
      }
    }
    auto set_tap = [&](int toff) {
#pragma unroll
      for (int i = 0; i < AI; ++i) {
        const bool in = a_base[i] >= 0 && (unsigned)(a_q[i] + toff) < (unsigned)g.segS;
        vA[i] = in ? a_base[i] + toff * (int)(g.lda * ESZ) : OOB;
      }
    };
    const int k_lo = kt_begin * BK, k_hi = (kt_begin + nk) * BK;
    const bool rotate = g.k_rot && g.taps == 1 && tiles_m > 1;
    int ld_k0 = k_lo + (rotate ? (int)((long)tm * nk / tiles_m) * BK : 0);
    int ld_c0 = ld_k0, ld_toff = g.tap0;
    if (kt_begin > 0 && !rotate) {
      const int tap = ld_k0 / g.tapC;
      ld_c0 = ld_k0 - tap * g.tapC;
      ld_toff = g.tap0 + tap * g.dil;
    }
    set_tap(ld_toff);
    auto issue = [&](int stage) {
      unsigned char* As = lds + stage * STAGE;
      unsigned char* Bs = As + BM * 128;
      const int sA = ld_c0 * ESZ, sW = ld_k0 * WSZ;
#pragma unroll
      for (int i = 0; i < AI; ++i) buf_lds16(g.A, g.a_bytes, As + (lw * AI + i) * 1024, vA[i], sA);
#pragma unroll
      for (int i = 0; i < BI; ++i) buf_lds16(g.W, g.w_bytes, Bs + (lw * BI + i) * 1024, vW[i], sW);
      ld_k0 += BK;
      ld_c0 += BK;
      if (rotate) {
        if (ld_k0 >= k_hi) ld_k0 = ld_c0 = k_lo;
      } else if (ld_c0 >= g.tapC) {
        ld_c0 = 0;
        ld_toff += g.dil;
        set_tap(ld_toff);
      }
    };
    const bool pstamp = g.dbg && (g.dbg_mode & 0xff) == 3 && lw == 0 && lane == 0;
    if (pstamp) g.dbg[(long)blockIdx.x * 4 + 0] = wall_clock64();
#pragma unroll
    for (int s = 0; s < NS - 1; ++s)
      if (s < nk) issue(s);
    if (pstamp) g.dbg[(long)blockIdx.x * 4 + 1] = wall_clock64();
    int stage = 0;
    const bool acct = g.dbg && (g.dbg_mode & 0xff) == 2 && lw == 0;
    long long t_mem = 0, t_bar = 0, t_start = acct ? (long long)__builtin_readcyclecounter() : 0;
// ... 143 lines not shown
      if (late) hard_barrier();
    }
    const unsigned char* As = lds + stage * STAGE;
    const unsigned char* Bs = As + BM * 128;
    auto reads = [&]() {
#pragma unroll
    for (int s = 0; s < 4; ++s) {
#pragma unroll
      for (int i = 0; i < FM; ++i) fa[s][i] = *(const bf16x8*)(As + a_row[i] + ((a_chunk(s) ^ a_sw[i]) << 4));
      if constexpr (WF == 0) {
#pragma unroll
        for (int j = 0; j < FN; ++j) fb[s][j] = *(const bf16x8*)(Bs + b_row[j] + ((a_chunk(s) ^ b_sw[j]) << 4));
      } else if (!(s & 1)) {
#pragma unroll
        for (int j = 0; j < FN; ++j) rawb[s >> 1][j] = *(const u32x4*)(Bs + b_row[j] + (((s + kh) ^ b_sw[j]) << 4));
      }
    }
    };
    reads();
    if (!late) {
      if constexpr (TWOB) {
        asm volatile("s_waitcnt lgkmcnt(0)" ::: "memory");
        hard_barrier();
      }
      cvtb();
      mma();
    }
    stage = stage + 1 == NS ? 0 : stage + 1;
  }
  if (late && nk > 0) cvtb();
  if (late && nk > 0) mma();
  }
  tl_stamp(g, 2);
  constexpr int XW = NW == 4 ? LW : 0;
  if constexpr (EPI == EPI_QKV_SPLIT) {
    gemm_epilogue_qkv<T, BM, BN, WM, WN, XW, NW == 4 && BM <= 128>(g, acc, lds, m0, n0);
  } else if constexpr (EPI == EPI_QKV_ATTN) {
    static_assert(NW == 4 && BM <= 128, "fused cross attention: four-consumer small tiles");
    gemm_epilogue_qkv<T, BM, BN, WM, WN, XW, true, true>(g, acc, lds, m0, n0);
  } else if constexpr (NW == 4) {
    gemm_epilogue_lds<T, EPI, BM, BN, WM, WN, XW>(g, acc, lds, m0, n0, ks);
  } else {
    if (g.vec_out) gemm_epilogue_lds<T, EPI, BM, BN, WM, WN, XW>(g, acc, lds, m0, n0, ks);
    else gemm_epilogue<T, EPI, FM, FN, TM, TN>(g, acc, m0, n0, wm, wn, fi, kh, ks);
  }
  tl_stamp(g, 3);
  if (g.dbg && (g.dbg_mode & 0xff) == 4 && tid == 0) g.dbg[(long)blockIdx.x * 4 + 3] = wall_clock64();
}

template <typename T, int BM, int BN, int WM, int WN, int NS, int LW, int EPI, int WF>
__global__ __launch_bounds__((WM * WN + LW) * 64) void gemm_ws_kernel(const GemmPair pr) {
  if ((int)blockIdx.x >= pr.tiles0) gemm_ws_body<T, BM, BN, WM, WN, NS, LW, EPI, WF, 1>(pr);
  else gemm_ws_body<T, BM, BN, WM, WN, NS, LW, EPI, WF, 0>(pr);
}

constexpr int conv3_inflight(int nsb, int tap, int ai, int bi) {
  int n = 0;
  for (int j = 1; j <= nsb - 2; ++j) n += bi + (((tap + j) % 3 == 0) ? ai : 0);
  return n;
}

template <typename T, int BM, int BN, int WM, int WN, int NSB, int NAB, int LW, int EPI, int WF>
__global__ __launch_bounds__((WM * WN + LW) * 64) void gemm_ws_conv3_kernel(const GemmPair pr) {
  const GemmArgs& g = pr.g[0];
  constexpr int NW = WM * WN;
  constexpr int BK = 64, ESZ = 2, OOB = 0x7ffffff0;
  constexpr int TM = BM / WM, TN = BN / WN, FM = TM / 32, FN = TN / 32;
  constexpr int WSZ = WF ? 1 : 2, BROW = 64 * WSZ;
  constexpr int APC = (BM + 2 + 7) / 8;
  constexpr int AI = (APC + LW - 1) / LW;
  constexpr int ABUF = AI * LW * 1024;
  constexpr int BI = BN * BROW / 1024 / LW;
  constexpr int BSL = BN * BROW;
  constexpr int ZOFF = NAB * ABUF + NSB * BSL;
  constexpr bool TWOB = BM >= 192 && BN == 128;
  static_assert(NW == 8 && (BN * BROW) % (1024 * LW) == 0 && BI >= 1, "bad tile");
  static_assert(3 * NAB >= NSB + 2, "an activation buffer would be refilled while its chunk is still being consumed");
  static_assert(conv3_inflight(NSB, 0, AI, BI) < 64 && conv3_inflight(NSB, 1, AI, BI) < 64 && conv3_inflight(NSB, 2, AI, BI) < 64,
                "vmcnt is a 6-bit counter");
  extern __shared__ __attribute__((aligned(16))) unsigned char lds[];

  const int tiles_m = (g.M + BM - 1) / BM;
  const int tiles_n = (g.N + BN - 1) / BN;
  int bid = (int)blockIdx.x;
  {
    const int nwg = tiles_m * tiles_n * (EPI == EPI_GATE_RES ? g.ksplit : 1);
    const int xcd = bid & 7, slot = bid >> 3;
    const int q = nwg >> 3, r = nwg & 7;
    bid = ((xcd < r) ? xcd * (q + 1) : r * (q + 1) + (xcd - r) * q) + slot;
  }
  int ks = 0;
  if constexpr (EPI == EPI_GATE_RES) {
    const int tiles = tiles_m * tiles_n;
    ks = bid / tiles;
    bid -= ks * tiles;
  }
  int tm, tn;
  tile_coords(bid, tiles_m, tiles_n, g.n_groups, tm, tn);
  const int m0 = tm * BM, n0 = tn * BN;
  const int tid = threadIdx.x, lane = tid & 63;
  const int wave = (BM == 256 && WF != 0) ? (tid >> 6) : __builtin_amdgcn_readfirstlane(tid >> 6);
  tl_stamp(g, 0);
  const int C = g.tapC;
  int kc_begin = 0, nkc = C / BK;
  if constexpr (EPI == EPI_GATE_RES) {
    const int tot = nkc;
    kc_begin = (int)((long)tot * ks / g.ksplit);
    nkc = (int)((long)tot * (ks + 1) / g.ksplit) - kc_begin;
  }
  const int nk = 3 * nkc;

  if (wave >= NW) {
    const int lw = wave - NW;
    const int lr = lane >> 3, lp = lane & 7;
    int vA[AI];
#pragma unroll
    for (int i = 0; i < AI; ++i) {
      const int j = (lw * AI + i) * 8 + lr;
      const int r = m0 - 1 + j;
      vA[i] = (j < BM + 2 && r >= 0 && r < g.M) ? (int)((unsigned)r * (unsigned)(g.lda * ESZ) + (unsigned)((lp ^ ((j >> 1) & 7)) * 16)) : OOB;
    }
    int vW[BI];
#pragma unroll
    for (int i = 0; i < BI; ++i) {
      if constexpr (WF == 0) {
        const int rl = (lw * BI + i) * 8 + lr;
        const int n = n0 + rl;
        vW[i] = (n < g.N) ? (int)((unsigned)n * (unsigned)(g.ldw * ESZ) + (unsigned)((lp ^ ((rl >> 1) & 7)) * 16)) : OOB;
      } else {
        const int rl = (lw * BI + i) * 16 + (lane >> 2);
        const int n = n0 + rl;
        vW[i] = (n < g.N) ? (int)((unsigned)n * (unsigned)g.ldw + (unsigned)(((lane & 3) ^ ((rl >> 2) & 3)) * 16)) : OOB;
      }
    }
    auto issue = [&](int sl) {
      const int c = sl / 3, tap = sl - 3 * c;
      const int ch = (kc_begin + c) * BK;
      if (tap == 0) {
        unsigned char* Ab = lds + (c % NAB) * ABUF;
#pragma unroll
        for (int i = 0; i < AI; ++i) buf_lds16(g.A, g.a_bytes, Ab + (lw * AI + i) * 1024, vA[i], ch * ESZ);
      }
      unsigned char* Bs = lds + NAB * ABUF + (sl % NSB) * BSL;
      const int sW = (tap * C + ch) * WSZ;
#pragma unroll
      for (int i = 0; i < BI; ++i) buf_lds16(g.W, g.w_bytes, Bs + (lw * BI + i) * 1024, vW[i], sW);
    };
#pragma unroll
    for (int sl = 0; sl < NSB - 1; ++sl)
      if (sl < nk) issue(sl);
    for (int kt0 = 0; kt0 < nk; kt0 += 3) {
#pragma unroll
      for (int tap = 0; tap < 3; ++tap) {
        const int kt = kt0 + tap;
        if (kt + NSB - 2 < nk) {
          if (tap == 0) asm volatile("s_waitcnt vmcnt(%0)" ::"n"(conv3_inflight(NSB, 0, AI, BI)) : "memory");
          else if (tap == 1) asm volatile("s_waitcnt vmcnt(%0)" ::"n"(conv3_inflight(NSB, 1, AI, BI)) : "memory");
          else asm volatile("s_waitcnt vmcnt(%0)" ::"n"(conv3_inflight(NSB, 2, AI, BI)) : "memory");
        } else {
          asm volatile("s_waitcnt vmcnt(0)" ::: "memory");
        }
        __builtin_amdgcn_s_barrier();
        if (kt + NSB - 1 < nk) issue(kt + NSB - 1);
        if constexpr (TWOB) __builtin_amdgcn_s_barrier();
      }
    }
    return;
  }

  const int wm = wave / WN, wn = wave % WN;
  const int fi = lane & 31, kh = lane >> 5;
  if (tid < 8) *(u32x4*)(lds + ZOFF + tid * 16) = u32x4{0u, 0u, 0u, 0u};
  f32x16 acc[FM][FN];
#pragma unroll
  for (int i = 0; i < FM; ++i)
#pragma unroll
    for (int j = 0; j < FN; ++j)
#pragma unroll
      for (int e = 0; e < 16; ++e) acc[i][j][e] = 0.f;
  int a_off[3][FM], a_swz[3][FM];
  bool a_ok[3][FM];
// ... 24 lines not shown
      for (int t = 0; t < 2; ++t)
#pragma unroll
        for (int j = 0; j < FN; ++j) cvt_fp8x16<WF, T>(rawb[t][j], fb[2 * t][j], fb[2 * t + 1][j]);
    }
  };
  auto mma = [&]() {
#pragma unroll
    for (int s = 0; s < 4; ++s)
#pragma unroll
      for (int i = 0; i < FM; ++i)
#pragma unroll
        for (int j = 0; j < FN; ++j)
          acc[i][j] = mfma16<T>(fa[s][i], fb[s][j], acc[i][j]);
  };
  const unsigned char* zrow = lds + ZOFF;
  for (int kt0 = 0; kt0 < nk; kt0 += 3) {
    const unsigned char* Ab = lds + ((kt0 / 3) % NAB) * ABUF;
#pragma unroll
    for (int tap = 0; tap < 3; ++tap) {
      const int kt = kt0 + tap;
      if (late) asm volatile("s_waitcnt lgkmcnt(0)" ::: "memory");
      if constexpr (TWOB) hard_barrier();
      else __builtin_amdgcn_s_barrier();
      if (kt == 0) tl_stamp(g, 1);
      if (late && kt > 0) {
        cvtb();
        mma();
      }
      if constexpr (TWOB) {
        if (late) hard_barrier();
      }
      const unsigned char* Bs = lds + NAB * ABUF + (kt % NSB) * BSL;
      auto reads = [&]() {
#pragma unroll
      for (int s = 0; s < 4; ++s) {
#pragma unroll
        for (int i = 0; i < FM; ++i) {
          const unsigned char* src = a_ok[tap][i] ? Ab + a_off[tap][i] + ((a_chunk(s) ^ a_swz[tap][i]) << 4) : zrow;
          fa[s][i] = *(const bf16x8*)src;
        }
        if constexpr (WF == 0) {
#pragma unroll
          for (int j = 0; j < FN; ++j) fb[s][j] = *(const bf16x8*)(Bs + b_row[j] + ((a_chunk(s) ^ b_sw[j]) << 4));
        } else if (!(s & 1)) {
#pragma unroll
          for (int j = 0; j < FN; ++j) rawb[s >> 1][j] = *(const u32x4*)(Bs + b_row[j] + (((s + kh) ^ b_sw[j]) << 4));
        }
      }
      };
      reads();
      if (!late) {
        if constexpr (TWOB) {
          asm volatile("s_waitcnt lgkmcnt(0)" ::: "memory");
          hard_barrier();
        }
        cvtb();
        mma();
      }
    }
  }
  if (late && nk > 0) {
    cvtb();
    mma();
  }
  tl_stamp(g, 2);
  if (g.vec_out) gemm_epilogue_lds<T, EPI, BM, BN, WM, WN>(g, acc, lds, m0, n0, ks);
  else gemm_epilogue<T, EPI, FM, FN, TM, TN>(g, acc, m0, n0, wm, wn, fi, kh, ks);
  tl_stamp(g, 3);
}

template <typename T, int EPI>
__global__ __launch_bounds__(768) void gemm_ws_conv3_ks_kernel(const GemmPair pr) {
  const GemmArgs& g = pr.g[0];
  constexpr int BM = 256, BN = 64, LW = 4, NSB = 6, NAB = 3, NW = 8;
  constexpr int BK = 64, ESZ = 2, OOB = 0x7ffffff0;
  constexpr int APC = (BM + 2 + 7) / 8, AI = (APC + LW - 1) / LW, ABUF = AI * LW * 1024;
  constexpr int BI = BN * 128 / 1024 / LW, BSL = BN * 128;
  constexpr int ZROW = 8 * APC;
  static_assert(ZROW + 8 <= AI * LW * 8, "the zero rows live in the surplus pieces of an activation buffer");
  extern __shared__ __attribute__((aligned(16))) unsigned char lds[];

  const int tiles_m = (g.M + BM - 1) / BM;
  const int tiles_n = (g.N + BN - 1) / BN;
  int bid = (int)blockIdx.x;
  {
    const int nwg = tiles_m * tiles_n * (EPI == EPI_GATE_RES ? g.ksplit : 1);
    const int xcd = bid & 7, slot = bid >> 3;
    const int q = nwg >> 3, r = nwg & 7;
    bid = ((xcd < r) ? xcd * (q + 1) : r * (q + 1) + (xcd - r) * q) + slot;
  }
  int ks = 0;
  if constexpr (EPI == EPI_GATE_RES) {
    const int tiles = tiles_m * tiles_n;
    ks = bid / tiles;
    bid -= ks * tiles;
  }
  int tm, tn;
  tile_coords(bid, tiles_m, tiles_n, g.n_groups, tm, tn);
  const int m0 = tm * BM, n0 = tn * BN;
  const int tid = threadIdx.x, lane = tid & 63;
  const int wave = __builtin_amdgcn_readfirstlane(tid >> 6);
  tl_stamp(g, 0);
  const int C = g.tapC;
  int kc_begin = 0, nkc = C / BK;
  if constexpr (EPI == EPI_GATE_RES) {
    const int tot = nkc;
    kc_begin = (int)((long)tot * ks / g.ksplit);
    nkc = (int)((long)tot * (ks + 1) / g.ksplit) - kc_begin;
  }
  const int nk = 3 * nkc;

  if (wave >= NW) {
    const int lw = wave - NW;
    const int lr = lane >> 3, lp = lane & 7;
    int vA[AI];
#pragma unroll
    for (int i = 0; i < AI; ++i) {
      const int j = (lw * AI + i) * 8 + lr;
      const int r = m0 - 1 + j;
      vA[i] = (j < BM + 2 && r >= 0 && r < g.M) ? (int)((unsigned)r * (unsigned)(g.lda * ESZ) + (unsigned)((lp ^ ((j >> 1) & 7)) * 16)) : OOB;
    }
    int vW[BI];
#pragma unroll
    for (int i = 0; i < BI; ++i) {
      const int rl = (lw * BI + i) * 8 + lr;
      const int n = n0 + rl;
      vW[i] = (n < g.N) ? (int)((unsigned)n * (unsigned)(g.ldw * ESZ) + (unsigned)((lp ^ ((rl >> 1) & 7)) * 16)) : OOB;
    }
    auto issue = [&](int sl) {
      const int c = sl / 3, tap = sl - 3 * c;
      const int ch = (kc_begin + c) * BK;
      if (tap == 0) {
        unsigned char* Ab = lds + (c % NAB) * ABUF;
#pragma unroll
        for (int i = 0; i < AI; ++i) buf_lds16(g.A, g.a_bytes, Ab + (lw * AI + i) * 1024, vA[i], ch * ESZ);
      }
      unsigned char* Bs = lds + NAB * ABUF + (sl % NSB) * BSL;
      const int sW = (tap * C + ch) * ESZ;
#pragma unroll
      for (int i = 0; i < BI; ++i) buf_lds16(g.W, g.w_bytes, Bs + (lw * BI + i) * 1024, vW[i], sW);
    };
#pragma unroll
    for (int sl = 0; sl < NSB - 1; ++sl)
      if (sl < nk) issue(sl);
    for (int kt0 = 0; kt0 < nk; kt0 += 3) {
#pragma unroll
      for (int tap = 0; tap < 3; ++tap) {
        const int kt = kt0 + tap;
        if (kt + NSB - 2 < nk) {
          if (tap == 0) asm volatile("s_waitcnt vmcnt(%0)" ::"n"(conv3_inflight(NSB, 0, AI, BI)) : "memory");
          else if (tap == 1) asm volatile("s_waitcnt vmcnt(%0)" ::"n"(conv3_inflight(NSB, 1, AI, BI)) : "memory");
          else asm volatile("s_waitcnt vmcnt(%0)" ::"n"(conv3_inflight(NSB, 2, AI, BI)) : "memory");
        } else {
          asm volatile("s_waitcnt vmcnt(0)" ::: "memory");
        }
        __builtin_amdgcn_s_barrier();
        if (kt + NSB - 1 < nk) issue(kt + NSB - 1);
      }
    }
    return;
  }

  const int wq = wave & 3, kq = wave >> 2;
  const int fi = lane & 31, kh = lane >> 5;
  f32x16 acc[2][2];
#pragma unroll
  for (int i = 0; i < 2; ++i)
#pragma unroll
    for (int j = 0; j < 2; ++j)
#pragma unroll
      for (int e = 0; e < 16; ++e) acc[i][j][e] = 0.f;
  int a_adr[3][2];
#pragma unroll
  for (int i = 0; i < 2; ++i) {
    const int tr = wq * 64 + i * 32 + fi;
    const int q = (m0 + tr) % g.segV;
#pragma unroll
    for (int t = 0; t < 3; ++t) {
      const bool ok = !((t == 0 && q == 0) || (t == 2 && q == g.segV - 1));
      const int j = ok ? tr + t : ZROW;
      a_adr[t][i] = j * 128 + (((4 * kq + 2 * kh) ^ ((j >> 1) & 7)) << 4);
// ... 314 lines not shown
```

### comfyui-hunyuanvideo-foley_amd/csrc/kernels.h

```cpp
#pragma once
#include "common.h"

enum GemmEpi {
  EPI_STORE_F32 = 0,
  EPI_STORE_T = 1,
  EPI_SILU_T = 2,
  EPI_GELU_T = 3,
  EPI_SILUGATE_T = 4,
  EPI_GATE_RES = 5,
  EPI_DAC = 6,
  EPI_QKV_SPLIT = 7,
  EPI_QKV_ATTN = 8,
  EPI_COUNT
};

struct QkvSplitArgs {
  const float* qkv;
  int M, L, H, nK;
  const float* gain[3];
  const int* pos[3];
  void* dst[3];
  int S_tot, tok_off;
  int out_dtype;
  int vt_pitch;
  float eps;
  const float* cos_tab;
  const float* sin_tab;
  const float* rcos[3];
  const float* rsin[3];
  const void* attn_k;
  const void* attn_vt;
  void* attn_out;
  int attn_skv, attn_pitch;
  int attn_bdiv;
  int* attn_fused;
};
struct GemmArgs {
  const void* A;
  const void* W;
  const float* bias;
  int M, N, K;
  long lda;
  long ldw;
  int segV, segS;
  int taps, tapC, dil, tap0;
  int rstride;
  void* out0;
  void* out1;
  int osegV;
  long out_seg, out_row, out_shift;
  int out_check;
  RowBcast rb;
  const float* res;
  const float* alpha;
  int alphaC;
  unsigned a_bytes, w_bytes;
  const void* zeros;
  int ksplit;
  float* partials;
  int partial_half;
  long partial_stride;
  int partial_cap;
  int n_groups;
  int k_rot;
  int krot_ok;
  QkvSplitArgs qs;
  int vec_out;
  int wfmt;
  int gelu_erf;
  int dbg_mode;
  long long* dbg;
};

int launch_gemm(const GemmArgs& g, int dtype, int epi, int tile, hipStream_t st, int* ksplit_used = nullptr);
int launch_gemm_pair(const GemmArgs& g0, const GemmArgs& g1, int dtype, int epi, hipStream_t st, int* ksplit_used = nullptr);
int launch_gemm_conv3(const GemmArgs& g, int dtype, int epi, int tile, hipStream_t st);
int launch_gemm_ws_bf16(const GemmArgs& g, const GemmArgs* g1, int epi, int tile, hipStream_t st);
int launch_gemm_ws_f16(const GemmArgs& g, const GemmArgs* g1, int epi, int tile, hipStream_t st);
int launch_gemm_wide_bf16(const GemmArgs& g, const GemmArgs* g1, int epi, int tile, hipStream_t st);
int launch_gemm_wide_f16(const GemmArgs& g, const GemmArgs* g1, int epi, int tile, hipStream_t st);

struct AttnArgs {
  const void* q;
  const void* k;
  const void* v;
  int Bq, H, Sq, Skv, kv_bdiv;
  void* outA;
  void* outB;
  int split;
  int in_dtype;
  int vt_pitch;
  int head_dim;
  long long* dbg;
  int grp_q, grp_kv;
  int out_nrows;
  const int* out_rows;
};
int launch_attention(const AttnArgs& a, int out_dtype, hipStream_t st);

struct AttnTimelineArgs {
  const void* q;
  const void* k;
  const void* v;
  const int* set_a;
  const int* set_b;
  const float* alpha;
  int Bq, H, Sq, Skv, n_sets;
  void* outA;
  void* outB;
  int split;
  int in_dtype;
  int vt_pitch;
};
int launch_attention_timeline(const AttnTimelineArgs& a, int out_dtype, hipStream_t st);

int launch_ln_mod(const float* x, int M, int D, float eps, const RowBcast& shift, const RowBcast& scale,
                  void* out, int out_dtype, hipStream_t st);
struct LnPending {
  const float* partials;
  int k;
  long stride;
  const float* bias;
  RowBcast gate;
  int half;
};
struct LnArgs {
  float* x;
  int M;
  RowBcast shift, scale;
  void* out;
  LnPending pend;
};
int launch_ln_mod_pending(float* x, int M, int D, float eps, const RowBcast& shift, const RowBcast& scale,
                          void* out, int out_dtype, const LnPending& pend, hipStream_t st);
int launch_ln_mod_pair(const LnArgs& a0, const LnArgs& a1, int D, float eps, int out_dtype, hipStream_t st);

int launch_qkv_split(const QkvSplitArgs& a, hipStream_t st);
int launch_qkv_split_pair(const QkvSplitArgs& a0, const QkvSplitArgs& a1, hipStream_t st);

int launch_rows_add_act(const float* a, const RowBcast& v, int R, int D, int act_silu, void* out,
                        int out_dtype, hipStream_t st);
int launch_rows_periodic_check(const float* x, int groups, int rows, int period, int D, int* flag, hipStream_t st);
int launch_add_periodic(const float* x, const float* pos, int R, int D, int period, void* out,
                        int out_dtype, hipStream_t st);
int launch_gather_rows(const float* src, const int* idx, int n_idx, int groups, int src_rows, int D,
                       float* out, hipStream_t st);
int launch_cast(const void* src, int src_dtype, void* dst, int dst_dtype, long n, hipStream_t st);

int launch_latent_rows(const float* x, int clips, int C, int L, int ncfg, void* out, int out_dtype,
                       hipStream_t st);

enum StepForm { STEP_FORM_PLAIN, STEP_FORM_EDIT, STEP_FORM_WINDOWS };
struct StepArgs {
  const float* pred;
  float* x;
  float* x_saved;
  float* d_acc;
  int clips, C, L, ncfg;
  float guidance;
  const float* coef;
  int* step_ptr;
  void* rows_out;
  int rows_dtype;
  const float* sched = nullptr;
  const float* clip_scale = nullptr;
  StepForm form = STEP_FORM_PLAIN;
  const float* x0 = nullptr;
  const float* noise = nullptr;
  const float* mask = nullptr;
  int x0_clips = 0, mask_clips = 0;
  int n_win = 0, Ltot = 0;
  const int* starts = nullptr;
  const float* weights = nullptr;
  float* hist = nullptr;
  int hist_slots = 0;
#pragma clang diagnostic push
#pragma clang diagnostic ignored "-Wc++20-extensions"
  bool operator==(const StepArgs&) const = default;
#pragma clang diagnostic pop
};
int launch_solver_step(const StepArgs& a, hipStream_t st);
// ... 39 lines not shown
```

Before: 15.05 audio-sec/sec.

## Prefetch next GEMM's weights into per-XCD L2 from spare attention workgroups

The single-stream self-attention launch gets extra workgroups when its grid is small. Those workgroups touch the 128-byte lines of the linear1 conv3 GEMM weight slices that each XCD will later read, so the weights are already in that XCD's L2 when the GEMM starts. A host planner works out which weight pieces each XCD will need from the GEMM tiling, and the tile-coordinate code is factored into a shared helper so planner and kernels agree. The cost is extra memory traffic and occupied CUs during attention, and the gain depends on the weights staying in L2 until the GEMM runs.

```diff
diff --git a/comfyui-hunyuanvideo-foley_amd/csrc/attention.hip b/comfyui-hunyuanvideo-foley_amd/csrc/attention.hip
--- a/comfyui-hunyuanvideo-foley_amd/csrc/attention.hip
+++ b/comfyui-hunyuanvideo-foley_amd/csrc/attention.hip
@@ -22,6 +22,41 @@
   b = bh / a.H;
 }
 
+__device__ __forceinline__ void attn_prefetch_role(const WeightPrefetch& d) {
+  const XcdPieces& xp = d.x[blockIdx.x & 7];
+  const int np = xp.n < PF_MAX_PIECES ? xp.n : PF_MAX_PIECES;
+  int total = 0;
+  for (int p = 0; p < np; ++p) total += xp.p[p].rows * ((xp.p[p].klen * d.es + 127) >> 7);
+  total = total < d.cap_lines ? total : d.cap_lines;
+  if (total <= 0) return;
+  const int stride = (d.n_wg >> 3) * 256;
+  const int first = ((((int)blockIdx.x - d.n_attn) >> 3) << 8) + (int)threadIdx.x;
+  auto line = [&](int l) {
+    l = l < total ? l : total - 1;
+    const WPiece& w0 = xp.p[0];
+    const char* adr = (const char*)d.W[w0.sel] + (long)w0.row0 * d.pitch[w0.sel] + (long)w0.k0 * d.es;
+    for (int p = 0; p < np; ++p) {
+      const WPiece& w = xp.p[p];
+      const int lpr = (w.klen * d.es + 127) >> 7, cnt = w.rows * lpr;
+      if ((unsigned)l < (unsigned)cnt) {
+        const int r = l / lpr;
+        adr = (const char*)d.W[w.sel] + (long)(w.row0 + r) * d.pitch[w.sel] + (long)w.k0 * d.es + ((l - r * lpr) << 7);
+      }
+      l -= cnt;
+    }
+    return *(const uint32_t*)adr;
+  };
+  uint32_t acc = 0;
+  for (int l = first; l < total; l += 8 * stride) {
+    uint32_t v[8];
+#pragma unroll
+    for (int u = 0; u < 8; ++u) v[u] = line(l + u * stride);
+#pragma unroll
+    for (int u = 0; u < 8; ++u) acc |= v[u];
+  }
+  asm volatile("" ::"v"(acc));
+}
+
 template <typename OutT> struct Pack4Out;
 template <> struct Pack4Out<float> {
   static __device__ __forceinline__ void store(float* p, const f32x4 v) { *(f32x4*)p = v; }
@@ -147,8 +182,16 @@
     }
 }
 
-template <typename T, typename OutT>
-__global__ __launch_bounds__(256) void attn_bf16_kernel(const AttnArgs a) {
+template <typename T, typename OutT, bool PF = false, typename... D>
+__global__ __launch_bounds__(256) void attn_bf16_kernel(const AttnArgs a, const D... pf) {
+  static_assert(sizeof...(D) == (PF ? 1 : 0), "the PF instances take one WeightPrefetch");
+  if constexpr (PF) {
+    const WeightPrefetch& d = (pf, ...);
+    if ((int)blockIdx.x >= d.n_attn) {
+      attn_prefetch_role(d);
+      return;
+    }
+  }
   constexpr int HD = 128;
   __shared__ float sO[4][3][16][64];
   __shared__ float sM[4][32], sL[4][32];
@@ -328,8 +371,16 @@
   __builtin_amdgcn_raw_ptr_buffer_load_lds(r, (__attribute__((address_space(3))) void*)lds_wave_base, 16, voff, 0, 0, 0);
 }
 
-template <typename T, typename OutT>
-__global__ __launch_bounds__(256) void attn_lds_kernel(const AttnArgs a, const int merge_off) {
+template <typename T, typename OutT, bool PF = false, typename... D>
+__global__ __launch_bounds__(256) void attn_lds_kernel(const AttnArgs a, const int merge_off, const D... pf) {
+  static_assert(sizeof...(D) == (PF ? 1 : 0), "the PF instances take one WeightPrefetch");
+  if constexpr (PF) {
+    const WeightPrefetch& d = (pf, ...);
+    if ((int)blockIdx.x >= d.n_attn) {
+      attn_prefetch_role(d);
+      return;
+    }
+  }
   constexpr int HD = 128;
   extern __shared__ __attribute__((aligned(16))) unsigned char dsm[];
   float (*sO)[3][16][64] = (float (*)[3][16][64])(dsm + merge_off);
@@ -1019,9 +1070,10 @@
 static long long* g_attn_dbg = nullptr;
 extern "C" void foley_debug_attn_timeline(void* p) { g_attn_dbg = (long long*)p; }
 
-int launch_attention(const AttnArgs& a_in, int out_dtype, hipStream_t st) {
+int launch_attention(const AttnArgs& a_in, int out_dtype, hipStream_t st, const WeightPrefetch* pf, int force) {
   AttnArgs a = a_in;
   a.dbg = g_attn_dbg;
+  if (pf && (pf->n_wg < 8 || (pf->n_wg & 7))) pf = nullptr;
   if (a.Sq <= 0 || a.Skv <= 0) return foley_set_err("attention: empty sequence", __FILE__, __LINE__);
   const int hd = a.head_dim > 0 ? a.head_dim : 128;
   if (hd != 128 && hd != 64 && hd != 96) return foley_set_err("attention: head_dim must be 128, 96 or 64", __FILE__, __LINE__);
@@ -1039,7 +1091,8 @@
     if (out_dtype != a.in_dtype && out_dtype != FOLEY_F32)
       return foley_set_err("attention: 16-bit operands produce the same type or fp32", __FILE__, __LINE__);
     const dim3 gw(((a.Sq + 127) / 128) * a.H * a.Bq);
-    const bool wide = (long)gw.x >= 256 || hd != 128, h16 = a.in_dtype == FOLEY_F16, o32 = out_dtype == FOLEY_F32;
+    if (force && (hd != 128 || a.grp_q > 0 || a.out_rows)) return foley_set_err("attention: the small-grid kernels serve head_dim 128", __FILE__, __LINE__);
+    const bool wide = !force && ((long)gw.x >= 256 || hd != 128), h16 = a.in_dtype == FOLEY_F16, o32 = out_dtype == FOLEY_F32;
     const bool longk = wide && hd == 128 && a.Skv >= 512 && (long)gw.x * 4 <= 2048;
     int pair_nq = 0;
     if (longk) {
@@ -1052,16 +1105,27 @@
     }
     const int nt = (a.Skv + 31) >> 5;
     const long img = (long)nt * 32 * 256 + (128L << ((a.vt_pitch > 128 ? 5 : 4) + 4)) + 32 * 256, mrg = 4 * 3 * 16 * 64 * 4 + 2 * 4 * 32 * 4;
-    const bool staged = !wide && hd == 128 && nt >= 4 && a.vt_pitch <= 256 && img <= 160 * 1024;
+    const bool staged = force ? force == 1 : !wide && hd == 128 && nt >= 4 && a.vt_pitch <= 256 && img <= 160 * 1024;
+    if (force == 1 && (a.vt_pitch > 256 || img > 160 * 1024)) return foley_set_err("attention: operands beyond the LDS-staged kernel", __FILE__, __LINE__);
+    WeightPrefetch pfd;
+    const bool ride = pf && !wide && (long)grid1.x + pf->n_wg <= 256;
+    if (ride) {
+      pfd = *pf;
+      pfd.n_attn = (int)grid1.x;
+    }
+    const dim3 grid_pf(grid1.x + (ride ? pfd.n_wg : 0));
     const int merge_off = staged && img + mrg <= 160 * 1024 ? (int)img : 0;
     const size_t lds16 = staged ? (size_t)(merge_off ? img + mrg : (img > mrg ? img : mrg)) : 0;
 #define FOLEY_ATTN16(T, O)                                                                         \
     do {                                                                                             \
       if (staged) {                                                                                  \
         static std::atomic<unsigned long long> raised{0};                                            \
-        hipError_t e_ = foley_raise_lds((const void*)attn_lds_kernel<T, O>, 160 * 1024, raised);     \
+        static std::atomic<unsigned long long> raised_pf{0};                                         \
+        hipError_t e_ = ride ? foley_raise_lds((const void*)attn_lds_kernel<T, O, true, WeightPrefetch>, 160 * 1024, raised_pf) \
+                             : foley_raise_lds((const void*)attn_lds_kernel<T, O>, 160 * 1024, raised); \
         if (e_ != hipSuccess) return foley_set_err(hipGetErrorString(e_), __FILE__, __LINE__);       \
-        FOLEY_LAUNCH((attn_lds_kernel<T, O>), grid1, dim3(256), lds16, st, a, merge_off);            \
+        if (ride) FOLEY_LAUNCH((attn_lds_kernel<T, O, true, WeightPrefetch>), grid_pf, dim3(256), lds16, st, a, merge_off, pfd); \
+        else FOLEY_LAUNCH((attn_lds_kernel<T, O>), grid1, dim3(256), lds16, st, a, merge_off);       \
       } else                                                                                         \
       if (pair_nq) {                                                                                 \
         static std::atomic<unsigned long long> r4{0}, r5{0}, r6{0};                                  \
@@ -1082,6 +1146,7 @@
       else if (wide && hd == 64) FOLEY_LAUNCH((attn_bf16_wide_kernel<T, O, 64>), gw, dim3(256), 0, st, a);  \
       else if (wide && hd == 96) FOLEY_LAUNCH((attn_bf16_wide_kernel<T, O, 96>), gw, dim3(256), 0, st, a);  \
       else if (wide) FOLEY_LAUNCH((attn_bf16_wide_kernel<T, O, 128>), gw, dim3(256), 0, st, a);        \
+      else if (ride) FOLEY_LAUNCH((attn_bf16_kernel<T, O, true, WeightPrefetch>), grid_pf, dim3(256), 0, st, a, pfd); \
       else FOLEY_LAUNCH((attn_bf16_kernel<T, O>), grid1, dim3(256), 0, st, a);                         \
     } while (0)
     if (h16) { if (o32) FOLEY_ATTN16(f16_t, float); else FOLEY_ATTN16(f16_t, f16_t); }
diff --git a/comfyui-hunyuanvideo-foley_amd/csrc/foley_rt.hip b/comfyui-hunyuanvideo-foley_amd/csrc/foley_rt.hip
--- a/comfyui-hunyuanvideo-foley_amd/csrc/foley_rt.hip
+++ b/comfyui-hunyuanvideo-foley_amd/csrc/foley_rt.hip
@@ -893,6 +893,24 @@
   } while (0)
 
 enum FwdPart { FWD_ALL = 0, FWD_HEAD, FWD_BODY, FWD_FINAL };
+
+constexpr int kPfWg = 64;
+constexpr long kPfCap = 0;
+static int g_pf_wg = kPfWg;
+static long g_pf_cap = kPfCap;
+static std::atomic<long> g_pf_launches{0};
+extern "C" void foley_debug_weight_prefetch(int wg, long cap) {
+  g_pf_wg = wg < 0 ? kPfWg : wg;
+  g_pf_cap = cap < 0 ? kPfCap : cap;
+}
+extern "C" long foley_debug_weight_prefetch_launches() { return g_pf_launches.load(); }
+static bool weight_prefetch_of(int dtype, const GemmArgs& g0, const GemmArgs* g1, int epi, WeightPrefetch& pf) {
+  bool ok = false;
+  if (dtype == FOLEY_BF16) ok = plan_weight_prefetch<bf16_t>(g0, g1, epi, g_pf_wg, g_pf_cap, pf);
+  else if (dtype == FOLEY_F16) ok = plan_weight_prefetch<f16_t>(g0, g1, epi, g_pf_wg, g_pf_cap, pf);
+  if (ok) g_pf_launches.fetch_add(1);
+  return ok;
+}
 
 static int run_forward(foley_ctx* c, hipStream_t st, FwdPart part = FWD_ALL) {
   const foley_config& f = c->cfg;
@@ -1076,13 +1094,13 @@
                            1.1920928955078125e-07f);
     PROF("single.qkv GEMM + RMSNorm/RoPE head split", gf(M, 3 * D, D), gb(M, 3 * D, D, es), launch_gemm(gq, T, EPI_QKV_SPLIT, 0, st));
     {
-      AttnArgs a{c->buf.Q, c->buf.K, c->buf.V, Bc, H, La, La, 1, c->buf.att_a, c->buf.att_a, 0, T, bf ? ly.Lap : 0};
-      PROF("single.self attention", af(Bc, La, La), ab(Bc, La, La), launch_attention(a, T, st));
-    }
-    {
       GemmArgs g = krot(gemm_conv(c->buf.att_a, M, La, D, 3, 1, w.lin1, c->buf.audio, D));
       g.rb = sm(2);
       with_partials(g, c->buf.part_a);
+      WeightPrefetch pf;
+      const bool ride = weight_prefetch_of(T, g, nullptr, EPI_GATE_RES, pf);
+      AttnArgs a{c->buf.Q, c->buf.K, c->buf.V, Bc, H, La, La, 1, c->buf.att_a, c->buf.att_a, 0, T, bf ? ly.Lap : 0};
+      PROF("single.self attention", af(Bc, La, La), ab(Bc, La, La), launch_attention(a, T, st, ride ? &pf : nullptr));
       int ks = 1;
       PROF("single.linear1 conv3 GEMM (gated residual)", gf(M, D, 3 * D), gb(M, D, 3 * D, 4), launch_gemm(g, T, EPI_GATE_RES, 0, st, &ks));
       if (ks > 1) pend[0] = LnPending{c->buf.part_a, ks, g.partial_stride, w.lin1.b, g.rb, slab_half};
@@ -1780,6 +1798,47 @@
   return 0;
 }
 
+extern "C" int foley_debug_weight_pieces(const foley_gemm_desc* d0, const foley_gemm_desc* d1, int single_clip, int xcd, int32_t* out) {
+  if (!out || xcd < 0 || xcd > 7) return FAIL(FOLEY_ERR_INVALID, "bad argument");
+  GemmArgs g0, g1;
+  if (int rc = d1 ? gemm_pair_args_of(d0, d1, g0, g1) : gemm_args_of(d0, g0)) return rc;
+  g0.krot_ok = g1.krot_ok = single_clip ? 1 : 0;
+  WeightPrefetch pf;
+  bool ok = false;
+  switch (d0->dtype) {
+    case FOLEY_F32: ok = plan_weight_prefetch<float>(g0, d1 ? &g1 : nullptr, d0->epilogue, 8, 0, pf); break;
+    case FOLEY_BF16: ok = plan_weight_prefetch<bf16_t>(g0, d1 ? &g1 : nullptr, d0->epilogue, 8, 0, pf); break;
+    case FOLEY_F16: ok = plan_weight_prefetch<f16_t>(g0, d1 ? &g1 : nullptr, d0->epilogue, 8, 0, pf); break;
+    default: return FAIL(FOLEY_ERR_INVALID, "GEMM: unsupported operand dtype");
+  }
+  out[0] = ok ? pf.x[xcd].n : 0;
+  for (int i = 0; i < out[0]; ++i) {
+    const WPiece& p = pf.x[xcd].p[i];
+    out[1 + 5 * i] = p.sel, out[2 + 5 * i] = p.row0, out[3 + 5 * i] = p.rows, out[4 + 5 * i] = p.k0, out[5 + 5 * i] = p.klen;
+  }
+  return 0;
+}
+
+extern "C" int foley_debug_attention_prefetch(const void* q, const void* k, const void* v, int in_dtype, int vt_pitch, int Bq, int H, int Sq,
+                                              int Skv, void* outA, void* outB, int split, int out_dtype, int kernel, const void* W, int wN,
+                                              int wK, int n_wg, void* stream) {
+  if (kernel != 1 && kernel != 2) return FAIL(FOLEY_ERR_INVALID, "kernel: 1 (LDS-staged) or 2 (register-loaded)");
+  AttnArgs a{q, k, v, Bq, H, Sq, Skv, 1, outA, outB, split, in_dtype, vt_pitch, 128};
+  if (n_wg < 0) return launch_attention(a, out_dtype, (hipStream_t)stream, nullptr, kernel);
+  if (n_wg < 8 || (n_wg & 7) || (W && (wN < 1 || wK < 2 || (wK & 1))))
+    return FAIL(FOLEY_ERR_INVALID, "prefetch workgroups: a multiple of 8; W: at least one row of an even number of elements");
+  WeightPrefetch pf{};
+  pf.W[0] = W, pf.pitch[0] = wK * 2, pf.es = 2, pf.n_wg = n_wg, pf.cap_lines = 0x7fffffff;
+  for (int x = 0; W && x < 8; ++x) {
+    const int r0 = (int)((long)wN * x / 8), r1 = (int)((long)wN * (x + 1) / 8);
+    if (r1 > r0) {
+      pf.x[x].n = 1;
+      pf.x[x].p[0] = WPiece{0, r0, r1 - r0, 0, wK};
+    }
+  }
+  return launch_attention(a, out_dtype, (hipStream_t)stream, &pf, kernel);
+}
+
 extern "C" int foley_op_attention_hd(const void* q, const void* k, const void* v, int in_dtype, int vt_pitch, int Bq,
                                      int H, int Sq, int Skv, int kv_bdiv, void* outA, void* outB, int split,
                                      int out_dtype, int head_dim, void* stream) {
diff --git a/comfyui-hunyuanvideo-foley_amd/csrc/gemm_conv3.hip b/comfyui-hunyuanvideo-foley_amd/csrc/gemm_conv3.hip
--- a/comfyui-hunyuanvideo-foley_amd/csrc/gemm_conv3.hip
+++ b/comfyui-hunyuanvideo-foley_amd/csrc/gemm_conv3.hip
@@ -1,4 +1,4 @@
-#include "gemm_common.h"
+#include "gemm_plan.h"
 
 namespace {
 
@@ -20,19 +20,8 @@
 
   const int tiles_m = (g.M + BM - 1) / BM;
   const int tiles_n = (g.N + BN - 1) / BN;
-  int bid = (int)blockIdx.x - (sel ? pr.tiles0 : 0);
-  {
-    const int nwg = tiles_m * tiles_n * (EPI == EPI_GATE_RES ? g.ksplit : 1);
-    const int xcd = bid & 7, slot = bid >> 3;
-    const int q = nwg >> 3, r = nwg & 7;
-    bid = ((xcd < r) ? xcd * (q + 1) : r * (q + 1) + (xcd - r) * q) + slot;
-  }
-  int ks = 0;
-  if constexpr (EPI == EPI_GATE_RES) {
-    ks = bid % g.ksplit;
-    bid /= g.ksplit;
-  }
-  const int tm = bid % tiles_m, tn = bid / tiles_m;
+  int tm, tn, ks;
+  wg_coords<EPI == EPI_GATE_RES, false>((int)blockIdx.x - (sel ? pr.tiles0 : 0), tiles_m, tiles_n, g.ksplit, 0, tm, tn, ks);
   const int m0 = tm * BM, n0 = tn * BN;
   const int tid = threadIdx.x, lane = tid & 63, wave = tid >> 6;
   tl_stamp(g, 0);
diff --git a/comfyui-hunyuanvideo-foley_amd/csrc/gemm_impl.h b/comfyui-hunyuanvideo-foley_amd/csrc/gemm_impl.h
--- a/comfyui-hunyuanvideo-foley_amd/csrc/gemm_impl.h
+++ b/comfyui-hunyuanvideo-foley_amd/csrc/gemm_impl.h
@@ -25,19 +25,8 @@
 
   const int tiles_m = (g.M + BM - 1) / BM;
   const int tiles_n = (g.N + BN - 1) / BN;
-  int bid = (int)blockIdx.x - (sel ? pr.tiles0 : 0);
-  {
-    const int nwg = tiles_m * tiles_n * (EPI == EPI_GATE_RES ? g.ksplit : 1);
-    const int xcd = bid & 7, slot = bid >> 3;
-    const int q = nwg >> 3, r = nwg & 7;
-    bid = ((xcd < r) ? xcd * (q + 1) : r * (q + 1) + (xcd - r) * q) + slot;
-  }
-  int ks = 0;
-  if constexpr (EPI == EPI_GATE_RES) {
-    ks = bid % g.ksplit;
-    bid /= g.ksplit;
-  }
-  const int tm = bid % tiles_m, tn = bid / tiles_m;
+  int tm, tn, ks;
+  wg_coords<EPI == EPI_GATE_RES, false>((int)blockIdx.x - (sel ? pr.tiles0 : 0), tiles_m, tiles_n, g.ksplit, 0, tm, tn, ks);
   const int m0 = tm * BM, n0 = tn * BN;
   const int tid = threadIdx.x, lane = tid & 63, wave = tid >> 6;
   tl_stamp(g, 0);
@@ -251,19 +240,8 @@
 
   const int tiles_m = (g.M + BM - 1) / BM;
   const int tiles_n = (g.N + BN - 1) / BN;
-  int bid = (int)blockIdx.x - (sel ? pr.tiles0 : 0);
-  {
-    const int nwg = tiles_m * tiles_n * (EPI == EPI_GATE_RES ? g.ksplit : 1);
-    const int xcd = bid & 7, slot = bid >> 3;
-    const int q = nwg >> 3, r = nwg & 7;
-    bid = ((xcd < r) ? xcd * (q + 1) : r * (q + 1) + (xcd - r) * q) + slot;
-  }
-  int ks = 0;
-  if constexpr (EPI == EPI_GATE_RES) {
-    ks = bid % g.ksplit;
-    bid /= g.ksplit;
-  }
-  const int tm = bid % tiles_m, tn = bid / tiles_m;
+  int tm, tn, ks;
+  wg_coords<EPI == EPI_GATE_RES, false>((int)blockIdx.x - (sel ? pr.tiles0 : 0), tiles_m, tiles_n, g.ksplit, 0, tm, tn, ks);
   const int m0 = tm * BM, n0 = tn * BN;
   const int tid = threadIdx.x, lane = tid & 63, wave = tid >> 6;
   tl_stamp(g, 0);
diff --git a/comfyui-hunyuanvideo-foley_amd/csrc/gemm_plan.h b/comfyui-hunyuanvideo-foley_amd/csrc/gemm_plan.h
--- a/comfyui-hunyuanvideo-foley_amd/csrc/gemm_plan.h
+++ b/comfyui-hunyuanvideo-foley_amd/csrc/gemm_plan.h
@@ -1,7 +1,56 @@
 #pragma once
 #include "gemm_common.h"
 
+#include <algorithm>
+#include <vector>
+
 namespace {
+
+
+__host__ __device__ __forceinline__ void tile_coords(int id, int tiles_m, int tiles_n, int n_groups, int& tm, int& tn) {
+  if (n_groups <= 0 || n_groups > tiles_n) {
+    tm = id % tiles_m;
+    tn = id / tiles_m;
+    return;
+  }
+  const int P = tiles_n / n_groups, r = tiles_n % n_groups;
+  const int big = r * (P + 1) * tiles_m;
+  int pg, p0, local;
+  if (id < big) {
+    pg = P + 1;
+    const int gi = id / (pg * tiles_m);
+    local = id - gi * pg * tiles_m;
+    p0 = gi * pg;
+  } else {
+    pg = P;
+    const int i2 = id - big, gi = i2 / (pg * tiles_m);
+    local = i2 - gi * pg * tiles_m;
+    p0 = r * (P + 1) + gi * pg;
+  }
+  tm = local / pg;
+  tn = p0 + local - tm * pg;
+}
+
+__host__ __device__ __forceinline__ int xcd_remap(int bid, int nwg) {
+  const int xcd = bid & 7, slot = bid >> 3;
+  const int q = nwg >> 3, r = nwg & 7;
+  return ((xcd < r) ? xcd * (q + 1) : r * (q + 1) + (xcd - r) * q) + slot;
+}
+
+template <bool SPLIT, bool MAJOR>
+__host__ __device__ __forceinline__ void wg_coords(int bid, int tiles_m, int tiles_n, int ksplit, int n_groups, int& tm, int& tn, int& ks) {
+  bid = xcd_remap(bid, tiles_m * tiles_n * (SPLIT ? ksplit : 1));
+  ks = 0;
+  if constexpr (SPLIT && MAJOR) {
+    const int tiles = tiles_m * tiles_n;
+    ks = bid / tiles;
+    bid -= ks * tiles;
+  } else if constexpr (SPLIT) {
+    ks = bid % ksplit;
+    bid /= ksplit;
+  }
+  tile_coords(bid, tiles_m, tiles_n, n_groups, tm, tn);
+}
 
 enum TileFamily : unsigned char { FAM_NONE, FAM_REG, FAM_GLDS, FAM_WS8, FAM_WS4, FAM_HEAD, FAM_CONV3, FAM_WSCONV3, FAM_WIDE };
 
@@ -309,4 +358,89 @@
   return plan;
 }
 
-}
+inline bool gemm_weight_pieces(const GemmPlan& plan, const GemmArgs& g0, const GemmArgs* g1, int epi, int xcd, std::vector<WPiece>& out) {
+  const TileInfo& ti = tile_info(plan.tile);
+  const bool conv = ti.fam == FAM_WSCONV3;
+  if (!(ti.fam == FAM_WS8 || ti.fam == FAM_WS4 || ti.fam == FAM_HEAD || conv) || (conv && g1)) return false;
+  constexpr int BK = 64;
+  const bool split = epi == EPI_GATE_RES;
+  const int ksp = split && plan.ksplit > 1 ? plan.ksplit : 1;
+  std::vector<WPiece> raw;
+  int first = 0;
+  for (int sel = 0; sel < (g1 ? 2 : 1); ++sel) {
+    const GemmArgs& q = sel ? *g1 : g0;
+    const int tiles_m = (q.M + ti.bm - 1) / ti.bm, tiles_n = (q.N + ti.bn - 1) / ti.bn;
+    const int nwg = tiles_m * tiles_n * ksp;
+    for (int bid = (xcd - first) & 7; bid < nwg; bid += 8) {
+      int tm, tn, ks;
+      if (split) wg_coords<true, true>(bid, tiles_m, tiles_n, ksp, plan.n_groups, tm, tn, ks);
+      else wg_coords<false, true>(bid, tiles_m, tiles_n, ksp, plan.n_groups, tm, tn, ks);
+      const int row0 = tn * ti.bn, rows = q.N - row0 < ti.bn ? q.N - row0 : ti.bn;
+      const int tot = (conv ? q.tapC : q.K) / BK;
+      const int b = (int)((long)tot * ks / ksp), e = (int)((long)tot * (ks + 1) / ksp);
+      if (e <= b) continue;
+      if (conv && e - b < tot)
+        for (int tap = 0; tap < q.taps; ++tap) raw.push_back(WPiece{sel, row0, rows, tap * q.tapC + b * BK, (e - b) * BK});
+      else
+        raw.push_back(WPiece{sel, row0, rows, b * BK, conv ? q.K : (e - b) * BK});
+    }
+    first += nwg;
+  }
+  std::sort(raw.begin(), raw.end(), [](const WPiece& a, const WPiece& b) {
+    if (a.sel != b.sel) return a.sel < b.sel;
+    if (a.k0 != b.k0) return a.k0 < b.k0;
+    if (a.klen != b.klen) return a.klen < b.klen;
+    return a.row0 < b.row0;
+  });
+  out.clear();
+  for (const WPiece& p : raw) {
+    if (!out.empty()) {
+      WPiece& l = out.back();
+      if (l.sel == p.sel && l.k0 == p.k0 && l.klen == p.klen && p.row0 <= l.row0 + l.rows) {
+        if (p.row0 + p.rows > l.row0 + l.rows) l.rows = p.row0 + p.rows - l.row0;
+        continue;
+      }
+    }
+    out.push_back(p);
+  }
+  return true;
+}
+
+template <typename T>
+bool plan_weight_prefetch(const GemmArgs& g0_in, const GemmArgs* g1_in, int epi, int n_wg, long cap_bytes, WeightPrefetch& pf) {
+  pf.n_wg = 0;
+  if constexpr (sizeof(T) != 2) return false;
+  n_wg &= ~7;
+  if (n_wg < 8 || !g0_in.krot_ok || !g0_in.W || (g1_in && !g1_in->W)) return false;
+  const GemmPlan plan = plan_gemm<T>(g0_in, g1_in, epi, 0, g0_in.krot_ok);
+  if (plan.err) return false;
+  GemmArgs g[2] = {g0_in, g1_in ? *g1_in : g0_in};
+  long total = 0;
+  for (int s = 0; s < (g1_in ? 2 : 1); ++s) {
+    if (g[s].ldw <= 0) g[s].ldw = g[s].K;
+    total += gemm_w_bytes<T>(g[s]);
+    pf.W[s] = g[s].W;
+  }
+  if (total > 24L << 20) return false;
+  pf.es = g[0].wfmt ? 1 : 2;
+  pf.pitch[0] = (int)(g[0].ldw * pf.es);
+  pf.pitch[1] = g1_in ? (int)(g[1].ldw * pf.es) : 0;
+  if (!g1_in) pf.W[1] = nullptr;
+  std::vector<WPiece> pieces;
+  for (int x = 0; x < 8; ++x) {
+    if (!gemm_weight_pieces(plan, g[0], g1_in ? &g[1] : nullptr, epi, x, pieces) || pieces.size() > (size_t)PF_MAX_PIECES) return false;
+    long bytes = 0;
+    pf.x[x].n = (int)pieces.size();
+    for (int i = 0; i < PF_MAX_PIECES; ++i) {
+      pf.x[x].p[i] = i < pf.x[x].n ? pieces[i] : WPiece{0, 0, 0, 0, 0};
+      bytes += (long)pf.x[x].p[i].rows * pf.x[x].p[i].klen * pf.es;
+    }
+    if (bytes > 3L << 20) return false;
+  }
+  pf.cap_lines = cap_bytes > 0 && cap_bytes / (8 * 128) < 0x7fffffffL ? (int)(cap_bytes / (8 * 128)) : 0x7fffffff;
+  pf.n_attn = 0;
+  pf.n_wg = n_wg;
+  return true;
+}
+
+}
diff --git a/comfyui-hunyuanvideo-foley_amd/csrc/gemm_wide_impl.h b/comfyui-hunyuanvideo-foley_amd/csrc/gemm_wide_impl.h
--- a/comfyui-hunyuanvideo-foley_amd/csrc/gemm_wide_impl.h
+++ b/comfyui-hunyuanvideo-foley_amd/csrc/gemm_wide_impl.h
@@ -35,21 +35,8 @@
 
   const int tiles_m = (g.M + BM - 1) / BM;
   const int tiles_n = (g.N + BN - 1) / BN;
-  int bid = (int)blockIdx.x - (SEL ? pr.tiles0 : 0);
-  {
-    const int nwg = tiles_m * tiles_n * (EPI == EPI_GATE_RES ? g.ksplit : 1);
-    const int xcd = bid & 7, slot = bid >> 3;
-    const int q = nwg >> 3, r = nwg & 7;
-    bid = ((xcd < r) ? xcd * (q + 1) : r * (q + 1) + (xcd - r) * q) + slot;
-  }
-  int ks = 0;
-  if constexpr (EPI == EPI_GATE_RES) {
-    const int tiles = tiles_m * tiles_n;
-    ks = bid / tiles;
-    bid -= ks * tiles;
-  }
-  int tm, tn;
-  tile_coords(bid, tiles_m, tiles_n, g.n_groups, tm, tn);
+  int tm, tn, ks;
+  wg_coords<EPI == EPI_GATE_RES, true>((int)blockIdx.x - (SEL ? pr.tiles0 : 0), tiles_m, tiles_n, g.ksplit, g.n_groups, tm, tn, ks);
   const int m0 = tm * BM, n0 = tn * BN;
   const int tid = threadIdx.x, lane = tid & 63;
   const int wave = __builtin_amdgcn_readfirstlane(tid >> 6);
diff --git a/comfyui-hunyuanvideo-foley_amd/csrc/gemm_ws_impl.h b/comfyui-hunyuanvideo-foley_amd/csrc/gemm_ws_impl.h
--- a/comfyui-hunyuanvideo-foley_amd/csrc/gemm_ws_impl.h
+++ b/comfyui-hunyuanvideo-foley_amd/csrc/gemm_ws_impl.h
@@ -4,37 +4,13 @@
 #include <type_traits>
 
 #include "common.h"
-#include "gemm_common.h"
+#include "gemm_plan.h"
 
 namespace {
 
 __device__ __forceinline__ void buf_lds16(const void* base, unsigned bytes, unsigned char* lds_wave_base, int voff, int soff) {
   const __amdgpu_buffer_rsrc_t r = __builtin_amdgcn_make_buffer_rsrc((void*)base, 0, (int)bytes, 0x00020000);
   __builtin_amdgcn_raw_ptr_buffer_load_lds(r, (__attribute__((address_space(3))) void*)lds_wave_base, 16, voff, soff, 0, 0);
-}
-
-__device__ __forceinline__ void tile_coords(int id, int tiles_m, int tiles_n, int n_groups, int& tm, int& tn) {
-  if (n_groups <= 0 || n_groups > tiles_n) {
-    tm = id % tiles_m;
-    tn = id / tiles_m;
-    return;
-  }
-  const int P = tiles_n / n_groups, r = tiles_n % n_groups;
-  const int big = r * (P + 1) * tiles_m;
-  int pg, p0, local;
-  if (id < big) {
-    pg = P + 1;
-    const int gi = id / (pg * tiles_m);
-    local = id - gi * pg * tiles_m;
-    p0 = gi * pg;
-  } else {
-    pg = P;
-    const int i2 = id - big, gi = i2 / (pg * tiles_m);
-    local = i2 - gi * pg * tiles_m;
-    p0 = r * (P + 1) + gi * pg;
-  }
-  tm = local / pg;
-  tn = p0 + local - tm * pg;
 }
 
 __device__ __forceinline__ void hard_barrier() {
@@ -90,21 +66,8 @@
 
   const int tiles_m = (g.M + BM - 1) / BM;
   const int tiles_n = (g.N + BN - 1) / BN;
-  int bid = (int)blockIdx.x - (sel ? pr.tiles0 : 0);
-  {
-    const int nwg = tiles_m * tiles_n * (EPI == EPI_GATE_RES ? g.ksplit : 1);
-    const int xcd = bid & 7, slot = bid >> 3;
-    const int q = nwg >> 3, r = nwg & 7;
-    bid = ((xcd < r) ? xcd * (q + 1) : r * (q + 1) + (xcd - r) * q) + slot;
-  }
-  int ks = 0;
-  if constexpr (EPI == EPI_GATE_RES) {
-    const int tiles = tiles_m * tiles_n;
-    ks = bid / tiles;
-    bid -= ks * tiles;
-  }
-  int tm, tn;
-  tile_coords(bid, tiles_m, tiles_n, g.n_groups, tm, tn);
+  int tm, tn, ks;
+  wg_coords<EPI == EPI_GATE_RES, true>((int)blockIdx.x - (sel ? pr.tiles0 : 0), tiles_m, tiles_n, g.ksplit, g.n_groups, tm, tn, ks);
   const int m0 = tm * BM, n0 = tn * BN;
   const int tid = threadIdx.x, lane = tid & 63;
   const int wave = __builtin_amdgcn_readfirstlane(tid >> 6);
@@ -414,21 +377,8 @@
 
   const int tiles_m = (g.M + BM - 1) / BM;
   const int tiles_n = (g.N + BN - 1) / BN;
-  int bid = (int)blockIdx.x;
-  {
-    const int nwg = tiles_m * tiles_n * (EPI == EPI_GATE_RES ? g.ksplit : 1);
-    const int xcd = bid & 7, slot = bid >> 3;
-    const int q = nwg >> 3, r = nwg & 7;
-    bid = ((xcd < r) ? xcd * (q + 1) : r * (q + 1) + (xcd - r) * q) + slot;
-  }
-  int ks = 0;
-  if constexpr (EPI == EPI_GATE_RES) {
-    const int tiles = tiles_m * tiles_n;
-    ks = bid / tiles;
-    bid -= ks * tiles;
-  }
-  int tm, tn;
-  tile_coords(bid, tiles_m, tiles_n, g.n_groups, tm, tn);
+  int tm, tn, ks;
+  wg_coords<EPI == EPI_GATE_RES, true>((int)blockIdx.x, tiles_m, tiles_n, g.ksplit, g.n_groups, tm, tn, ks);
   const int m0 = tm * BM, n0 = tn * BN;
   const int tid = threadIdx.x, lane = tid & 63;
   const int wave = (BM == 256 && WF != 0) ? (tid >> 6) : __builtin_amdgcn_readfirstlane(tid >> 6);
@@ -619,21 +569,8 @@
 
   const int tiles_m = (g.M + BM - 1) / BM;
   const int tiles_n = (g.N + BN - 1) / BN;
-  int bid = (int)blockIdx.x;
-  {
-    const int nwg = tiles_m * tiles_n * (EPI == EPI_GATE_RES ? g.ksplit : 1);
-    const int xcd = bid & 7, slot = bid >> 3;
-    const int q = nwg >> 3, r = nwg & 7;
-    bid = ((xcd < r) ? xcd * (q + 1) : r * (q + 1) + (xcd - r) * q) + slot;
-  }
-  int ks = 0;
-  if constexpr (EPI == EPI_GATE_RES) {
-    const int tiles = tiles_m * tiles_n;
-    ks = bid / tiles;
-    bid -= ks * tiles;
-  }
-  int tm, tn;
-  tile_coords(bid, tiles_m, tiles_n, g.n_groups, tm, tn);
+  int tm, tn, ks;
+  wg_coords<EPI == EPI_GATE_RES, true>((int)blockIdx.x, tiles_m, tiles_n, g.ksplit, g.n_groups, tm, tn, ks);
   const int m0 = tm * BM, n0 = tn * BN;
   const int tid = threadIdx.x, lane = tid & 63;
   const int wave = __builtin_amdgcn_readfirstlane(tid >> 6);
diff --git a/comfyui-hunyuanvideo-foley_amd/csrc/kernels.h b/comfyui-hunyuanvideo-foley_amd/csrc/kernels.h
--- a/comfyui-hunyuanvideo-foley_amd/csrc/kernels.h
+++ b/comfyui-hunyuanvideo-foley_amd/csrc/kernels.h
@@ -96,7 +96,22 @@
   int out_nrows;
   const int* out_rows;
 };
-int launch_attention(const AttnArgs& a, int out_dtype, hipStream_t st);
+constexpr int PF_MAX_PIECES = 8;
+struct WPiece { int sel, row0, rows, k0, klen; };
+struct XcdPieces {
+  int n;
+  WPiece p[PF_MAX_PIECES];
+};
+struct WeightPrefetch {
+  const void* W[2];
+  int pitch[2];
+  int es;
+  int n_wg;
+  int n_attn;
+  int cap_lines;
+  XcdPieces x[8];
+};
+int launch_attention(const AttnArgs& a, int out_dtype, hipStream_t st, const WeightPrefetch* pf = nullptr, int force = 0);
 
 struct AttnTimelineArgs {
   const void* q;
```

New measurement: 15.06 audio-sec/sec (median of 2 runs). About the same (+0.1%).
